# facebook/transform360

Hardware: NVIDIA H100
Metric: Mpixels/s 8K equirect->cubemap bicubic (input-plane pixels consumed per second) (higher is better)
Workload: dtype u8

## Files before the change

### include/transform360_b200.h

```cpp
#ifndef TRANSFORM360_B200_EXT_H
#define TRANSFORM360_B200_EXT_H

#include "Transform360/VideoFrameTransformHandler.h"

#ifdef __cplusplus
extern "C" {
#endif

typedef struct T360HostPlan T360HostPlan;

T360HostPlan* T360B200_hostPlanCreate(const FrameTransformContext* ctx, int inputWidth, int inputHeight,
                                      int outputWidth, int outputHeight);
#define T360_BORDER_WRAP 3
#define T360_BORDER_TRANSPARENT 5
T360HostPlan* T360B200_hostPlanCreateFromWarp(const FrameTransformContext* ctx, const float* map, int mapWidth, int mapHeight,
                                              int inputWidth, int inputHeight, int border);
void T360B200_hostPlanDestroy(T360HostPlan* plan);
int T360B200_hostPlanInfo(const T360HostPlan* plan, int info[6]);
const float* T360B200_hostPlanMap(const T360HostPlan* plan);
const int32_t* T360B200_hostPlanSamples(const T360HostPlan* plan);
int T360B200_hostPlanGather(T360HostPlan* plan, int info[10], const int32_t** jobs, const int32_t** records,
                            const uint32_t** compact);
int T360B200_hostPlanPoleCaps(T360HostPlan* plan, int info[4], const int32_t** capJobs, const uint32_t** capRecords,
                              const int32_t** launchJobs);
int T360B200_dealLanes(int interpolationAlg, int n, const int32_t* phases, int32_t* laneOf, int32_t* copyOf);
int T360B200_weightImage(int interpolationAlg, const uint8_t** image);
int T360B200_hostPlanBlurLists(T360HostPlan* const* plans, int numPlans, int width, int height, int layout[15],
                               const uint8_t** image);
int T360B200_hostPlanSegment(const T360HostPlan* plan, int i, int rect[4], int numTaps[2], const float** kx,
                             const float** ky);
int T360B200_remapTable(int interpolationAlg, const int16_t** table);

int T360B200_generateMapFromWarp(VideoFrameTransform* transform, const float* map, int mapWidth, int mapHeight, int inputWidth,
                                 int inputHeight, int border, int transformMatPlaneIndex);
int T360B200_remapFrameAsync(VideoFrameTransform* transform, int numPlanes, const float* const* deviceMaps, const int* mapPitches,
                             int border, const uint8_t* const* deviceInputs, uint8_t* const* deviceOutputs, const int* inputWidths,
                             const int* inputHeights, const int* inputPitches, const int* outputWidths, const int* outputHeights,
                             const int* outputPitches, void* cudaStream);

int T360B200_transformFramePlaneAsync(VideoFrameTransform* transform, const uint8_t* deviceInput,
                                      uint8_t* deviceOutput, int inputWidth, int inputHeight, int inputPitch,
                                      int outputWidth, int outputHeight, int outputPitch,
                                      int transformMatPlaneIndex, void* cudaStream);
int T360B200_transformFrameAsync(VideoFrameTransform* transform, int numPlanes, const uint8_t* const* deviceInputs,
                                 uint8_t* const* deviceOutputs, const int* inputWidths, const int* inputHeights,
                                 const int* inputPitches, const int* outputWidths, const int* outputHeights,
                                 const int* outputPitches, void* cudaStream);
int T360B200_lowPassPlaneAsync(VideoFrameTransform* transform, const uint8_t* deviceInput, uint8_t* deviceOutput,
                               int width, int height, int inputPitch, int outputPitch,
                               int transformMatPlaneIndex, void* cudaStream);
int T360B200_reconfigure(VideoFrameTransform* transform, const FrameTransformContext* ctx);
int T360B200_reconfigureAsync(VideoFrameTransform* transform, const FrameTransformContext* ctx);
int T360B200_reconfigureWait(VideoFrameTransform* transform, int block);
typedef struct T360View {
  float yaw, pitch, hfov, vfov;
} T360View;
int T360B200_transformFrameViewAsync(VideoFrameTransform* transform, const T360View* view, int numPlanes,
                                     const uint8_t* const* deviceInputs, uint8_t* const* deviceOutputs, const int* inputWidths,
                                     const int* inputHeights, const int* inputPitches, const int* outputWidths,
                                     const int* outputHeights, const int* outputPitches, void* cudaStream);
int T360B200_viewSamples(const FrameTransformContext* ctx, const T360View* view, int inputWidth, int inputHeight,
                         int outputWidth, int outputHeight, int32_t* samples);
typedef struct T360Orientation {
  float yaw, pitch, roll;
} T360Orientation;
int T360B200_transformFrameOrientedAsync(VideoFrameTransform* transform, const T360Orientation* orientation, int numPlanes,
                                         const uint8_t* const* deviceInputs, uint8_t* const* deviceOutputs,
                                         const int* inputWidths, const int* inputHeights, const int* inputPitches,
                                         const int* outputWidths, const int* outputHeights, const int* outputPitches,
                                         void* cudaStream);
int T360B200_orientedSamples(const FrameTransformContext* ctx, const T360Orientation* orientation, int inputWidth,
                             int inputHeight, int outputWidth, int outputHeight, int32_t* samples);
typedef struct T360Pose {
  float yaw, pitch, roll, hfov, vfov;
} T360Pose;
int T360B200_transformFramePoseAsync(VideoFrameTransform* transform, const T360Pose* pose, int numPlanes,
                                     const uint8_t* const* deviceInputs, uint8_t* const* deviceOutputs, const int* inputWidths,
                                     const int* inputHeights, const int* inputPitches, const int* outputWidths,
                                     const int* outputHeights, const int* outputPitches, void* cudaStream);
int T360B200_poseSamples(const FrameTransformContext* ctx, const T360Pose* pose, int inputWidth, int inputHeight,
                         int outputWidth, int outputHeight, int32_t* samples);
typedef struct T360Lens {
  float fx, fy, cx, cy;
  float k[4];
  float yaw, pitch, roll;
  float maxAngle;
} T360Lens;
typedef struct T360LensRig {
  int numLenses, calibWidth, calibHeight;
  T360Lens lens[2];
} T360LensRig;
int T360B200_lensMap(const FrameTransformContext* ctx, const T360LensRig* rig, const T360Orientation* orientation, int inputWidth,
                     int inputHeight, int outputWidth, int outputHeight, float* map);
int T360B200_transformFrameLensAsync(VideoFrameTransform* transform, const T360LensRig* rig, const T360Orientation* orientation,
                                     int numPlanes, const uint8_t* const* deviceInputs, uint8_t* const* deviceOutputs,
                                     const int* inputWidths, const int* inputHeights, const int* inputPitches,
                                     const int* outputWidths, const int* outputHeights, const int* outputPitches, void* cudaStream);
void T360B200_setPinHostPlanes(VideoFrameTransform* transform, int enable);
void T360B200_debugTrace(VideoFrameTransform* transform, int enable);
unsigned long long T360B200_debugTraceRead(VideoFrameTransform* transform, unsigned long long* out, unsigned long long maxWords);
int T360B200_synchronize(VideoFrameTransform* transform);
void* T360B200_stream(VideoFrameTransform* transform);

unsigned long long T360B200_kernelLaunchCount(void);
unsigned long long T360B200_planDeviceBytes(VideoFrameTransform* transform, int transformMatPlaneIndex);
int T360B200_planTileCounts(VideoFrameTransform* transform, int transformMatPlaneIndex, int counts[4]);
int T360B200_deviceCount(void);
const char* T360B200_version(void);

#ifdef __cplusplus
}
#endif
#endif
```

### transform360_b200/csrc/gather_frame.cu

```cuda
#include "gather_common.cuh"

#include <cuda.h>

#include <algorithm>
#include <cstring>
#include <utility>

namespace t360 {

namespace {

template <class F, int... I>
__device__ __forceinline__ void staticForImpl(F&& f, std::integer_sequence<int, I...>) {
  (f(std::integral_constant<int, I>{}), ...);
}
template <int N, class F>
__device__ __forceinline__ void staticFor(F&& f) {
  staticForImpl(f, std::make_integer_sequence<int, N>{});
}

template <int IMM>
__device__ __forceinline__ uint32_t ldsWordImm(uint32_t addr) {
  uint32_t v;
  asm volatile("ld.shared.u32 %0, [%1+%2];" : "=r"(v) : "r"(addr), "n"(IMM));
// ... 80 lines not shown
  }
  return acc;
}
template <int K>
__device__ __forceinline__ uint32_t slotOffset(uint32_t field) { return K == 2 ? field >> 1 : field; }

template <int VS>
__device__ __forceinline__ int foldRowsRotated(const RowBytes<8> (&W)[8], uint32_t wAddr, uint32_t field) {
  static_assert(VS == 16384, "one copy of the table");
  const uint32_t r = ((field >> 4) ^ threadIdx.x) & 7u;
  const uint32_t first = field ^ (r * (uint32_t)kDiagonalStep);
  const bool p0 = (r & 1u) != 0, p1 = (r & 2u) != 0, p2 = (r & 4u) != 0;
  RowBytes<8> A[8], B[8];
#pragma unroll
  for (int i = 0; i < 8; ++i)
#pragma unroll
    for (int h = 0; h < 2; ++h) A[i].b[h] = p0 ? W[i ^ 1].b[h] : W[i].b[h];
#pragma unroll
  for (int i = 0; i < 8; ++i)
#pragma unroll
    for (int h = 0; h < 2; ++h) B[i].b[h] = p1 ? A[i ^ 2].b[h] : A[i].b[h];
  int acc = 1 << 14;
  staticFor<8>([&](auto V) {
    constexpr int v = decltype(V)::value;
    const uint4 wt = ldsVecImm<0>(wAddr + (first ^ (uint32_t)(v * kDiagonalStep)));
    const uint32_t b0 = p2 ? B[v ^ 4].b[0] : B[v].b[0], b1 = p2 ? B[v ^ 4].b[1] : B[v].b[1];
    acc = dp2aLo(wt.x, b0, acc); acc = dp2aHi(wt.y, b0, acc);
    acc = dp2aLo(wt.z, b1, acc); acc = dp2aHi(wt.w, b1, acc);
  });
  return acc;
}
template <int K, int VS>
__device__ __forceinline__ int foldPixel(const RowBytes<K> (&W)[K], uint32_t wAddr, uint32_t field) {
  if constexpr (K == 8) return foldRowsRotated<VS>(W, wAddr, field);
  else return foldRows<K, VS>(W, wAddr + slotOffset<K>(field));
}
__device__ __forceinline__ int biasedToByte(int acc) { return min(max(acc >> 15, 0), 255); }


__device__ __forceinline__ uint32_t packBytes(int hi, int lo) {
  uint32_t r;
  asm("cvt.pack.sat.u8.s32.b32 %0, %1, %2, %3;" : "=r"(r) : "r"(hi), "r"(lo), "r"(0));
  return r;
}

template <int K, int PITCH, int VS, int ROWS, bool ZERO>
__device__ __forceinline__ void computeShareJob(uint8_t* dst, int dstPitch, uint32_t stageAddr, const uint4 (&rec)[ROWS / 8],
                                                uint32_t header, uint32_t wAddr) {
  static_assert(PITCH % 4 == 0 && (K == 4 || K == 8) && ROWS % 8 == 0, "");
  uint32_t base = stageAddr + (header & 0x7ffcu);
  const int sh = (int)(header << 3);
  RowBytes<K> W[K];
  staticFor<K>([&](auto R) { W[decltype(R)::value] = loadRow<K, decltype(R)::value * PITCH>(base, sh); });
  int accPrev = 0;
  staticFor<ROWS>([&](auto J) {
    constexpr int j = decltype(J)::value;
    const uint4& block = rec[j >> 3];
    const uint32_t word = ((j >> 1) & 3) == 0 ? block.x : (((j >> 1) & 3) == 1 ? block.y : (((j >> 1) & 3) == 2 ? block.z : block.w));
    const uint32_t r = (j & 1) ? word >> 16 : word;
    if constexpr (j > 0 && !ZERO) {
      const bool two = (r & 1u) != 0;
      const RowBytes<K> below = loadRow<K, (j - 1 + K) * PITCH>(base, sh);
      RowBytes<K> below2 = below;
      if (two) below2 = loadRow<K, (j + K) * PITCH>(base, sh);
#pragma unroll
      for (int q = 0; q + 2 < K; ++q)
#pragma unroll
        for (int i = 0; i < (K == 8 ? 2 : 1); ++i) W[q].b[i] = two ? W[q + 2].b[i] : W[q + 1].b[i];
#pragma unroll
      for (int i = 0; i < (K == 8 ? 2 : 1); ++i) W[K - 2].b[i] = two ? below.b[i] : W[K - 1].b[i];
      W[K - 1] = below2;
      if (two) base += PITCH;
    }
    if constexpr (j > 0 && ZERO) {
      const uint32_t d = r & 3u;
      RowBytes<K> below = W[K - 1], below2 = W[K - 1];
      if (d != 0) below = loadRow<K, K * PITCH>(base, sh);
      if (d == 2) below2 = loadRow<K, (K + 1) * PITCH>(base, sh);
#pragma unroll
      for (int q = 0; q + 2 < K; ++q)
#pragma unroll
        for (int i = 0; i < (K == 8 ? 2 : 1); ++i) W[q].b[i] = d == 0 ? W[q].b[i] : (d == 1 ? W[q + 1].b[i] : W[q + 2].b[i]);
#pragma unroll
      for (int i = 0; i < (K == 8 ? 2 : 1); ++i) {
        W[K - 2].b[i] = d == 0 ? W[K - 2].b[i] : (d == 1 ? W[K - 1].b[i] : below.b[i]);
        W[K - 1].b[i] = d == 0 ? W[K - 1].b[i] : (d == 1 ? below.b[i] : below2.b[i]);
      }
      base += d * PITCH;
    }
    const int acc = foldPixel<K, VS>(W, wAddr, r & kSlotFieldMask) >> 15;
    if constexpr (j & 1) {
      const uint32_t pair = packBytes(acc, accPrev);
      dst[(size_t)(j - 1) * dstPitch] = (uint8_t)pair;
      dst[(size_t)j * dstPitch] = (uint8_t)(pair >> 8);
    } else {
      accPrev = acc;
    }
  });
}

template <int K, int PITCH, int VS>
__device__ __forceinline__ void computeTileJob(const PlaneView& pv, uint32_t stageAddr, int outX, int outY, const uint4& rec,
                                               uint32_t wAddr, int warp) {
  static_assert(PITCH % 4 == 0, "");
  const int y0 = outY + warp * kTilePatchH;
  const int dstPitch = pv.dstPitch, dstW = pv.dstW, dstH = pv.dstH;
  uint8_t* const dstRow = pv.dst + (size_t)y0 * dstPitch + outX;
  const uint32_t words[4] = {rec.x, rec.y, rec.z, rec.w};
  staticFor<kRowsPerPatchStep>([&](auto J) {
    constexpr int j = decltype(J)::value;
    const uint32_t w = words[j];
    const int col = kTilePatchW * j + ((int)(w >> 16) & (kTilePatchW - 1)), row = (int)(w >> 19) & (kTilePatchH - 1);
    if (!(w & kRecordSkip) && outX + col < dstW && y0 + row < dstH) {
      const uint32_t rowAddr = stageAddr + (w & 0x7ffcu);
      const int sh = (int)(w << 3);
      RowBytes<K> W[K];
      staticFor<K>([&](auto R) { W[decltype(R)::value] = loadRow<K, decltype(R)::value * PITCH>(rowAddr, sh); });
      const int acc = foldPixel<K, VS>(W, wAddr, (w >> 17) & kSlotFieldMask);
      dstRow[(size_t)row * dstPitch + col] = (uint8_t)biasedToByte(acc);
    }
  });
}

template <int K, int PITCH, int VS>
__device__ __forceinline__ void computeCapJob(const PlaneView& pv, uint32_t stageAddr, uint32_t recAddr, int steps, uint32_t wAddr,
                                              int warp, int lane) {
  static_assert(PITCH % 4 == 0, "");
  for (int s = warp; s < steps; s += kGroupWarps) {
    const uint2 r = ldsVec2Imm<0>(recAddr + s * kCapStepBytes + lane * 8);
    if (r.x & kRecordSkip) continue;
    const uint32_t rowAddr = stageAddr + (r.x & 0x7ffcu);
    const int sh = (int)(r.x << 3);
    RowBytes<K> W[K];
    staticFor<K>([&](auto R) { W[decltype(R)::value] = loadRow<K, decltype(R)::value * PITCH>(rowAddr, sh); });
    const int acc = foldPixel<K, VS>(W, wAddr, (r.x >> 17) & kSlotFieldMask);
    pv.dst[(size_t)(r.y >> 16) * pv.dstPitch + (r.y & 0xffffu)] = (uint8_t)biasedToByte(acc);
  }
}

template <int K, int VS>
__device__ __forceinline__ void computeBorderJob(const PlaneView& pv, uint32_t recAddr, int n, const unsigned char* wsmem, int warp, int lane) {
  SrcView sv;
  sv.bytes = pv.src;
  sv.misalign = (int)(reinterpret_cast<uintptr_t>(pv.src) & 3);
  sv.words = reinterpret_cast<const uint32_t*>(pv.src - sv.misalign);
  sv.w = pv.srcW; sv.h = pv.srcH; sv.pitch = pv.srcPitch;
  for (int i = warp * 32 + lane; i < n; i += kGroupThreads) {
    const uint4 r = ldsVecImm<0>(recAddr + i * kBorderPixelBytes);
    const int v = gatherPixel<K, false, VS, weightDiagonal(K)>(sv, wsmem, (int)r.x, (int)r.y);
    pv.dst[(size_t)(r.z >> 16) * pv.dstPitch + (r.z & 0xffffu)] = (uint8_t)v;
  }
}

struct FrameTensorMaps {
  CUtensorMap map[kMaxFramePlanes][kNumBoxClasses][kBoxVariants];
};

__device__ __forceinline__ void mbarArrive(uint64_t* bar) {
  asm volatile("mbarrier.arrive.shared::cta.b64 _, [%0];" ::"r"(smemAddr(bar)) : "memory");
}
__device__ __forceinline__ uint4 ldsVec(uint32_t addr) {
  uint4 v;
  asm volatile("ld.shared.v4.u32 {%0, %1, %2, %3}, [%4];" : "=r"(v.x), "=r"(v.y), "=r"(v.z), "=r"(v.w) : "r"(addr));
  return v;
}
__device__ __forceinline__ uint32_t ldsWord(uint32_t addr) {
  uint32_t v;
  asm volatile("ld.shared.u32 %0, [%1];" : "=r"(v) : "r"(addr));
  return v;
}

template <int K, int COPIES, int GROUPS>
struct FrameLayout {
  static constexpr int kStages = gatherStages(K);
  static constexpr int kWeights = weightImageBytes(K, COPIES);
  static constexpr int kStage = stageBytesOf(K), kRec = stageRecordBytes(K);
  static constexpr int kGroupBytes = kStages * (kStage + kRec);
  static constexpr int kPlanes = kWeights + GROUPS * kGroupBytes;
  static constexpr int kBars = kPlanes + 256;
  static constexpr int kTotal = kBars + GROUPS * kStages * 16 + 16;
  static_assert(kTotal <= 232448, "227 KB of shared memory per CTA");
  static_assert(sizeof(PlaneView) * kMaxFramePlanes <= 256, "");
  static_assert(kStage % 128 == 0 && kRec % 128 == 0 && kWeights % 128 == 0, "TMA / bulk-copy destinations");
};

template <int K, int COPIES, int GROUPS>
__global__ void __launch_bounds__(GROUPS * (kGroupWarps + 1) * 32, 1)
gatherFrameKernel(const __grid_constant__ FrameGatherParams p, StagedParams jobs, const __grid_constant__ FrameTensorMaps maps) {
  using L = FrameLayout<K, COPIES, GROUPS>;
  constexpr int VS = weightVectorStride(K, COPIES), kStage = L::kStage, kRec = L::kRec, S = L::kStages;
  constexpr uint32_t kBox0 = stageBoxW(K, 0) * stageBoxH(K, 0), kBox1 = stageBoxW(K, 1) * stageBoxH(K, 1),
                     kBoxShare = stageBoxW(K, 2) * stageBoxH(K, 2);
  static_assert(kBox1 + 64 <= 2 * kStage && kBox0 + 64 <= kStage && kBoxShare + 64 <= kStage, "boxes must fit their stage buffers");
  static_assert(boxVariantRows(K, 0, kBoxVariants - 1) > 0 && boxVariantRows(K, 2, kBoxVariants - 1) > 0, "");
  extern __shared__ __align__(128) unsigned char smem[];
  unsigned char* wsmem = smem;
  PlaneView* planes = reinterpret_cast<PlaneView*>(smem + L::kPlanes);
  uint64_t* barBase = reinterpret_cast<uint64_t*>(smem + L::kBars);
  uint64_t* weightBar = barBase + GROUPS * 2 * S;
  const int warpId = threadIdx.x >> 5, lane = threadIdx.x & 31;
  constexpr int kProducerWarp = GROUPS * kGroupWarps;

  asm volatile("griddepcontrol.launch_dependents;" ::: "memory");
  if (threadIdx.x == 0) {
    for (int g = 0; g < GROUPS; ++g)
      for (int st = 0; st < S; ++st) {
        mbarInit(barBase + g * 2 * S + st, 1);
        mbarInit(barBase + g * 2 * S + S + st, kGroupWarps);
      }
    mbarInit(weightBar, 1);
    asm volatile("fence.mbarrier_init.release.cluster;" ::: "memory");
  }
  if (threadIdx.x < kMaxFramePlanes * (int)(sizeof(PlaneView) / 4))
    reinterpret_cast<uint32_t*>(planes)[threadIdx.x] = reinterpret_cast<const uint32_t*>(p.plane)[threadIdx.x];
  __syncthreads();

  if (warpId >= kProducerWarp) {
    const int g = warpId - kProducerWarp;
    if (g == 0 && lane == 0) {
      mbarExpectTx(weightBar, L::kWeights);
      constexpr int kChunk = L::kWeights / 4;
      for (int i = 0; i < 4; ++i)
        bulkCopyToShared(wsmem + i * kChunk, reinterpret_cast<const unsigned char*>(p.weightImage) + i * kChunk, kChunk, weightBar);
    }
    const int producer = blockIdx.x * GROUPS + g, dynamicBase = gridDim.x * GROUPS * 2 * kClaimBatch;
    auto loadBatch = [&](int base) {
      int4 h = make_int4(0, kJobExit << kJobKindShift, 0, 0);
      if (lane < kClaimBatch && base + lane < jobs.numTiles) h = __ldg(reinterpret_cast<const int4*>(jobs.tiles) + base + lane);
      return h;
    };
    int4 batch = loadBatch(producer * 2 * kClaimBatch);
    int4 batchNext = loadBatch((producer * 2 + 1) * kClaimBatch);
    asm volatile("griddepcontrol.wait;" ::: "memory");
    int claimed = 0;
    if (lane == 0) claimed = atomicAdd(jobs.claimCounter, kClaimBatch);
    unsigned char* groupBase = smem + L::kWeights + g * L::kGroupBytes;
    uint64_t* full = barBase + g * 2 * S;
    uint64_t* empty = full + S;
    int pos = 0;
    uint32_t st = 0, phase = 0;
    auto advance = [&]() { if (++st == S) { st = 0; phase ^= 1; } };
    auto postEmptyJob = [&](int kind) {
      *reinterpret_cast<int4*>(groupBase + S * kStage + st * kRec) = make_int4(0, kind << kJobKindShift, 0, 0);
      mbarArrive(full + st);
    };
    for (;;) {
      if (pos == kClaimBatch) {
        batch = batchNext;
        pos = 0;
        batchNext = loadBatch(dynamicBase + __shfl_sync(0xffffffffu, claimed, 0));
        if (lane == 0) claimed = atomicAdd(jobs.claimCounter, kClaimBatch);
      }
      int4 h;
      h.x = __shfl_sync(0xffffffffu, batch.x, pos); h.y = __shfl_sync(0xffffffffu, batch.y, pos);
      h.z = __shfl_sync(0xffffffffu, batch.z, pos); h.w = __shfl_sync(0xffffffffu, batch.w, pos);
      ++pos;
      const int kind = (h.y >> kJobKindShift) & kJobKindMask;
      mbarWait(empty + st, phase ^ 1);
      const bool twoStages = kind == kJobClass1 || kind == kJobSeam;
      if (twoStages) {
        if (st == S - 1) {
          if (lane == 0) postEmptyJob(kJobNop);
          advance();
          mbarWait(empty + st, phase ^ 1);
        }
        mbarWait(empty + st + 1, phase ^ 1);
      }
      if (lane == 0) {
        unsigned char* rec = groupBase + S * kStage + st * kRec;
        *reinterpret_cast<int4*>(rec) = h;
        if (kind == kJobExit) {
          mbarArrive(full + st);
        } else {
          const int pl = h.y >> kJobPlaneShift;
          const uint32_t recBytes = (uint32_t)jobRecordBytes(K, kind, h.x);
          if (kind == kJobBorder) {
            mbarExpectTx(full + st, recBytes);
          } else {
            const int cls = boxClassOf(kind), variant = jobBoxVariant(h.z), boxX = jobBoxX(h.z), boxY = jobBoxY(h.z);
            const uint32_t boxBytes = (uint32_t)(stageBoxW(K, cls) * boxVariantRows(K, cls, variant));
            mbarExpectTx(full + st, (kind == kJobSeam ? 2 : 1) * boxBytes + recBytes);
            tmaLoadBox(groupBase + st * kStage, &maps.map[pl][cls][variant], boxX, boxY, full + st);
            if (kind == kJobSeam)
              tmaLoadBox(groupBase + (st + 1) * kStage, &maps.map[pl][0][variant], boxX - planes[pl].srcW, boxY, full + st);
          }
          bulkCopyToShared(rec + 128, planes[pl].records + (unsigned)h.w, recBytes, full + st);
        }
      }
      advance();
      if (twoStages) {
        if (lane == 0) postEmptyJob(kJobNop);
        advance();
      }
      __syncwarp();
      if (kind == kJobExit) break;
    }
    if (lane == 0 && atomicAdd(jobs.claimCounter + 1, 1) == (int)(gridDim.x * GROUPS) - 1) {
      jobs.claimCounter[0] = 0;
      jobs.claimCounter[1] = 0;
      __threadfence();
    }
    return;
  }

  const int group = warpId / kGroupWarps, warp = warpId % kGroupWarps;
  unsigned char* groupBase = smem + L::kWeights + group * L::kGroupBytes;
  const uint32_t boxAddr = smemAddr(groupBase), recAddr = smemAddr(groupBase + S * kStage);
  uint64_t* full = barBase + group * 2 * S;
  uint64_t* empty = full + S;
  const uint32_t wAddr = smemAddr(wsmem);
  mbarWait(weightBar, 0);
  asm volatile("griddepcontrol.wait;" ::: "memory");
  auto now = []() { unsigned long long t; asm volatile("mov.u64 %0, %globaltimer;" : "=l"(t)); return t; };
  unsigned long long* trace = jobs.trace && warp == 0 && lane == 0 ? jobs.trace + (size_t)(blockIdx.x * GROUPS + group) * kTraceJobsPerGroup * 4 : nullptr;
  uint32_t traced = 0;
  for (uint32_t st = 0, phase = 0;;) {
    unsigned long long* const row = trace && traced < kTraceJobsPerGroup ? trace + traced * 4 : nullptr;
    if (row) row[0] = now();
    mbarWait(full + st, phase);
    if (row) row[1] = now();
    const uint32_t rec = recAddr + st * kRec;
    const uint4 h = ldsVec(rec);
    const int kind = ((int)h.y >> kJobKindShift) & kJobKindMask;
    if (kind == kJobExit) break;
    const int outX = (int)h.x & ~kJobQuadMask, outY = (int)h.y & kJobRowMask;
    const PlaneView& pv = planes[(int)h.y >> kJobPlaneShift];
    if (kind == kJobShare || kind == kJobShareStay) {
      if constexpr (K >= 4) {
        const uint32_t mine = rec + 128 + warp * shareWarpRecordBytes(K);
        uint4 r[shareRows(K) / 8];
#pragma unroll
        for (int b = 0; b < shareRows(K) / 8; ++b) r[b] = ldsVec(mine + b * 512 + lane * 16);
        const uint32_t header = ldsWord(mine + shareRows(K) / 8 * 512 + lane * 4);
        uint8_t* dst = pv.dst + (size_t)(outY + (warp >> 1) * shareRows(K)) * pv.dstPitch + (outX + (warp & 1) * 32 + (int)(header >> kRecordColumnShift));
        if (kind == kJobShare) computeShareJob<K, stageBoxW(K, 2), VS, shareRows(K), false>(dst, pv.dstPitch, boxAddr + st * kStage, r, header, wAddr);
        else computeShareJob<K, stageBoxW(K, 2), VS, shareRows(K), true>(dst, pv.dstPitch, boxAddr + st * kStage, r, header, wAddr);
      }
    } else if (kind == kJobClass0) {
      uint4 r;
      const int quad = ((int)h.x & kJobQuadMask) - 1;
      if (quad < 0) {
        r = ldsVec(rec + 128 + warp * 512 + lane * 16);
      } else {
        r = make_uint4(kRecordSkip, kRecordSkip, kRecordSkip, kRecordSkip);
        if ((warp >> 2) == (quad >> 1)) {
          const uint2 v = ldsVec2Imm<0>(rec + 128 + (warp & 3) * 256 + lane * 8);
          if (quad & 1) { r.z = v.x; r.w = v.y; } else { r.x = v.x; r.y = v.y; }
        }
      }
      computeTileJob<K, stageBoxW(K, 0), VS>(pv, boxAddr + st * kStage, outX, outY, r, wAddr, warp);
    } else if (kind == kJobClass1) {
      computeTileJob<K, stageBoxW(K, 1), VS>(pv, boxAddr + st * kStage, outX, outY, ldsVec(rec + 128 + warp * 512 + lane * 16), wAddr, warp);
    } else if (kind == kJobSeam) {
      {
        uint4* a = reinterpret_cast<uint4*>(groupBase + st * kStage);
        const uint4* b = reinterpret_cast<const uint4*>(groupBase + (st + 1) * kStage);
        for (int i = warp * 32 + lane; i < (int)(kBox0 / 16); i += kGroupThreads) {
          uint4 x = a[i];
          const uint4 y = b[i];
          x.x |= y.x; x.y |= y.y; x.z |= y.z; x.w |= y.w;
          a[i] = x;
        }
        asm volatile("fence.proxy.async.shared::cta;" ::: "memory");
      }
      groupBarrier(group);
      computeTileJob<K, stageBoxW(K, 0), VS>(pv, boxAddr + st * kStage, outX, outY, ldsVec(rec + 128 + warp * 512 + lane * 16), wAddr, warp);
    } else if (kind == kJobCap) {
      computeCapJob<K, stageBoxW(K, 0), VS>(pv, boxAddr + st * kStage, rec + 128, (int)h.x, wAddr, warp, lane);
    } else if (kind == kJobBorder) {
      computeBorderJob<K, VS>(pv, rec + 128, (int)h.x, wsmem, warp, lane);
    }
    __syncwarp();
    if (lane == 0) mbarArrive(empty + st);
    if (row) {
      row[2] = now(); row[3] = kind;
      ++traced;
    }
    if (++st == S) { st = 0; phase ^= 1; }
  }
}

template <int K, int COPIES, int GROUPS>
cudaError_t prepareFrameK(LaunchCfg& cfg) {
  static DeviceLaunchCfg cfgs;
  constexpr int threads = GROUPS * (kGroupWarps + 1) * 32, smemBytes = FrameLayout<K, COPIES, GROUPS>::kTotal;
  return prepare<gatherFrameKernel<K, COPIES, GROUPS>>(cfgs, threads, smemBytes, cfg);
}

template <int K, int COPIES, int GROUPS>
cudaError_t launchFrameK(const FrameGatherParams& p, const StagedParams& jobs, const FrameTensorMaps& maps, int numSMs,
                         cudaStream_t stream, bool programmatic) {
  constexpr int threads = GROUPS * (kGroupWarps + 1) * 32, smemBytes = FrameLayout<K, COPIES, GROUPS>::kTotal;
  LaunchCfg cfg;
  cudaError_t err = prepareFrameK<K, COPIES, GROUPS>(cfg);
  if (err != cudaSuccess) return err;
  const int grid = std::min(numSMs * cfg.perSM, (jobs.numTiles + GROUPS * 2 * kClaimBatch - 1) / (GROUPS * 2 * kClaimBatch));
  cudaLaunchConfig_t lc{};
  lc.gridDim = dim3(grid);
  lc.blockDim = dim3(threads);
  lc.dynamicSmemBytes = smemBytes;
  lc.stream = stream;
  cudaLaunchAttribute attr{};
  attr.id = cudaLaunchAttributeProgrammaticStreamSerialization;
  attr.val.programmaticStreamSerializationAllowed = 1;
  lc.attrs = &attr;
  lc.numAttrs = programmatic ? 1 : 0;
  err = cudaLaunchKernelEx(&lc, gatherFrameKernel<K, COPIES, GROUPS>, p, jobs, maps);
  gLaunches.fetch_add(1, std::memory_order_relaxed);
  return err;
}

}

cudaError_t prepareGatherFrame(int kernelSize) {
  LaunchCfg cfg;
  switch (kernelSize) {
    case 2: return prepareFrameK<2, weightCopies(2), gatherGroups(2)>(cfg);
    case 4: return prepareFrameK<4, weightCopies(4), gatherGroups(4)>(cfg);
    case 8: return prepareFrameK<8, weightCopies(8), gatherGroups(8)>(cfg);
    default: return cudaErrorInvalidValue;
  }
}

cudaError_t launchGatherFrame(const FrameGatherParams& p, const StagedParams& jobs, const void* tensorMaps, int numSMs,
                              cudaStream_t stream, bool programmatic) {
  if (jobs.numTiles <= 0) return cudaSuccess;
  if (p.numPlanes < 1 || p.numPlanes > kMaxFramePlanes) return cudaErrorInvalidValue;
  FrameTensorMaps maps;
  std::memcpy(&maps, tensorMaps, sizeof(CUtensorMap) * kNumBoxClasses * kBoxVariants * p.numPlanes);
  for (int i = p.numPlanes; i < kMaxFramePlanes; ++i)
    for (int c = 0; c < kNumBoxClasses; ++c)
      for (int v = 0; v < kBoxVariants; ++v) maps.map[i][c][v] = maps.map[0][c][v];
  switch (p.kernelSize) {
    case 2: return launchFrameK<2, weightCopies(2), gatherGroups(2)>(p, jobs, maps, numSMs, stream, programmatic);
    case 4: return launchFrameK<4, weightCopies(4), gatherGroups(4)>(p, jobs, maps, numSMs, stream, programmatic);
    case 8: return launchFrameK<8, weightCopies(8), gatherGroups(8)>(p, jobs, maps, numSMs, stream, programmatic);
    default: return cudaErrorInvalidValue;
  }
}

}
```

### transform360_b200/csrc/gather_plan.cpp

```cpp
#include "gather_plan.h"

#include <algorithm>
#include <climits>
#include <cstdint>
#include <cstring>
#include <stdexcept>
#include <thread>
#include <utility>

namespace t360 {
namespace {

template <class F>
void parallelRanges(int n, size_t workPerItem, F fn) {
  unsigned nt = std::thread::hardware_concurrency();
  if (nt == 0) nt = 1;
  if (nt > 32) nt = 32;
  if (static_cast<size_t>(n) * workPerItem < (1u << 16)) nt = 1;
  const int chunk = (n + static_cast<int>(nt) - 1) / static_cast<int>(nt);
  std::vector<std::thread> pool;
  for (unsigned t = 1; t < nt; ++t) {
    const int b = static_cast<int>(t) * chunk, e = std::min(n, b + chunk);
    if (b < e) pool.emplace_back(fn, b, e);
  }
// ... 433 lines not shown
    return false;
  }
  bool deal(const int* load) {
    std::memset(share, 0, sizeof(share));
    std::fill(fill, fill + 4, 0);
    for (int g = 0; g < groups; ++g)
      for (int i = 0; i < load[g]; ++i) {
        std::fill(seen, seen + 4, false);
        if (!put(g)) return false;
      }
    return true;
  }
};

int dealLanes(int k, int copies, int n, const int* slot, int* laneOf, int* copyOf) {
  const int groups = weightBankGroups(k), lanesPerPass = weightLanesPerPass(k), passes = 32 / lanesPerPass;
  for (int i = 0; i < n; ++i) { laneOf[i] = i; copyOf[i] = 0; }
  if (n < 32) return 0;
  int group[32];
  if (copies > 1 && groups == 8) {
    int base[32];
    for (int i = 0; i < n; ++i) base[i] = slot[i] & 7;
    GroupMatcher m{n, copies, 0, base, {}, {}, {}};
    for (m.cap = 4; m.cap <= 32; ++m.cap)
      if (m.run()) break;
    m.balance();
    for (int i = 0; i < n; ++i) {
      group[i] = m.groupOf[i];
      copyOf[i] = (m.groupOf[i] - base[i]) & 7;
    }
  } else {
    for (int i = 0; i < n; ++i) group[i] = slot[i] & (groups - 1);
  }
  int load[16] = {};
  for (int i = 0; i < n; ++i) ++load[group[i]];
  int share[16][4] = {}, height[4] = {};
  {
    int fullest = 0;
    for (int g = 0; g < groups; ++g) fullest = std::max(fullest, load[g]);
    PassDealer d{groups, passes, lanesPerPass, {}, {}, {}, {}};
    bool done = false;
    for (int total = std::max(passes, fullest); !done; ++total) {
      int h[4] = {1, 1, 1, 1};
      auto tryHeights = [&]() {
        std::copy(h, h + 4, d.h);
        if (!d.deal(load)) return false;
        std::memcpy(share, d.share, sizeof(share));
        std::copy(h, h + 4, height);
        return true;
      };
      if (passes == 2) {
        for (h[1] = total / 2; h[1] >= 1 && !done; --h[1]) { h[0] = total - h[1]; done = tryHeights(); }
      } else {
        for (h[3] = total / 4; h[3] >= 1 && !done; --h[3])
          for (h[2] = (total - h[3]) / 3; h[2] >= h[3] && !done; --h[2])
            for (h[1] = (total - h[3] - h[2]) / 2; h[1] >= h[2] && !done; --h[1]) {
              h[0] = total - h[3] - h[2] - h[1];
              done = tryHeights();
            }
      }
    }
  }
  int nextLane[4];
  for (int q = 0; q < passes; ++q) nextLane[q] = q * lanesPerPass;
  for (int g = 0; g < groups; ++g) {
    int q = 0;
    for (int i = 0; i < n; ++i) {
      if (group[i] != g) continue;
      while (share[g][q] == 0) ++q;
      --share[g][q];
      laneOf[i] = nextLane[q]++;
    }
  }
  int wavefronts = 0;
  for (int q = 0; q < passes; ++q) wavefronts += height[q];
  return wavefronts;
}

std::vector<uint8_t> buildWeightImage(int k, const int16_t* table) {
  const int copies = weightCopies(k);
  std::vector<uint8_t> img(static_cast<size_t>(weightImageBytes(k, copies)), 0);
  for (int phase = 0; phase < 1024; ++phase) {
    const int slot = weightSlotOf(k, phase);
    const int16_t* cell = table + static_cast<size_t>(phase) * k * k;
    if (k == 2) {
      std::memcpy(&img[static_cast<size_t>(slot) * 8], cell, 8);
      continue;
    }
    for (int c = 0; c < copies; ++c)
      for (int v = 0; v < k * k / 8; ++v)
        std::memcpy(&img[static_cast<size_t>(weightVectorOffset(k, copies, (weightSlotInCopy(slot, c) << 4) | (c << 14), v))], cell + v * 8, 16);
  }
  return img;
}

void buildGatherPlan(const HostPlan& h, bool stageTiles, GatherPlan& g) {
  g = GatherPlan{};
  const int k = h.kernelSize;
  if (k <= 0) return;
  g.tileH = gatherTileH(k);
  g.tilesPerRow = (h.mapW + kGatherTileW - 1) / kGatherTileW;
  g.tileRows = (h.mapH + g.tileH - 1) / g.tileH;
  g.records.assign(static_cast<size_t>(g.tilesPerRow) * g.tileRows * g.tileH * kGatherTileW, int2{0, 0});
  buildFullRecords(h, g.records, g.tilesPerRow, g.tileH);
  if (!stageTiles) return;

  const int tilesX = g.tilesPerRow, tilesY = (h.mapH + kFrameTileH - 1) / kFrameTileH;
  const bool seamPossible = h.inW % 16 == 0 && h.inW >= 4 * stageBoxW(k, 0);
  std::vector<TileClass> cls(static_cast<size_t>(tilesX) * tilesY);
  const int blockRows = shareH(k) / kFrameTileH;
  parallelRanges((tilesY + blockRows - 1) / blockRows, static_cast<size_t>(h.mapW) * shareH(k), [&](int byBegin, int byEnd) {
    for (int by = byBegin; by < byEnd; ++by)
      for (int tx = 0; tx < tilesX; tx += 2) {
        TileClass* c = &cls[static_cast<size_t>(by) * blockRows * tilesX + tx];
        if (shareBlock(h, tx * 32, by * shareH(k), c[0])) continue;
        for (int ty = by * blockRows; ty < std::min(tilesY, (by + 1) * blockRows); ++ty)
          for (int t = tx; t < std::min(tilesX, tx + 2); ++t)
            classifyTile(h, t * 32, ty * kFrameTileH, seamPossible, cls[static_cast<size_t>(ty) * tilesX + t]);
      }
  });

  for (int ty = 0; ty < tilesY; ++ty)
    for (int tx = 0; tx < tilesX; ++tx) {
      const TileClass& c = cls[static_cast<size_t>(ty) * tilesX + tx];
      const int kind = c.kind;
      if (kind < 0) continue;
      for (int q = 0; q < (c.quads ? 4 : 1); ++q) {
        GatherJob job{tx * 32, ty * kFrameTileH | (kind << kJobKindShift),
                      kind == kJobGeneral ? 0 : jobBoxField(c.boxX, c.boxY, boxVariantFor(k, boxClassOf(kind), c.boxRows)), 0};
        if (c.quads) {
          job.outX |= q + 1;
          job.boxXY = jobBoxField(c.quadBoxX[q], c.quadBoxY[q], boxVariantFor(k, 0, c.quadBoxRows[q]));
        }
        g.jobs.push_back(job);
      }
      switch (kind) {
        case kJobGeneral: ++g.numGeneral; break;
        case kJobSeam: ++g.numSeam; break;
        case kJobShare: case kJobShareStay: ++g.numShare; break;
        default: g.numStaged[kind] += c.quads ? 4 : 1; break;
      }
    }
  std::stable_sort(g.jobs.begin(), g.jobs.end(), [](const GatherJob& a, const GatherJob& b) { return jobLaunchRank(a) < jobLaunchRank(b); });
  size_t offset = 0;
  for (GatherJob& job : g.jobs) {
    const int kind = (job.outY >> kJobKindShift) & kJobKindMask;
    if (kind == kJobGeneral) continue;
    job.recordOffset = static_cast<int>(offset / 16);
    offset += jobRecordBytes(k, kind, job.outX);
  }
  g.compact.assign(offset / 4, 0u);
  std::vector<int> needRows(g.jobs.size(), h.inH);
  std::vector<JobRect> rects(g.jobs.size());
  parallelRanges(static_cast<int>(g.jobs.size()), 2048, [&](int begin, int end) {
    for (int i = begin; i < end; ++i) {
      const GatherJob& job = g.jobs[i];
      JobRect& r = rects[i];
      r = tileRect(job, k);
      r.x1 = std::min(r.x1, h.mapW);
      r.y1 = std::min(r.y1, h.mapH);
      const int kind = (job.outY >> kJobKindShift) & kJobKindMask;
      if (kind == kJobGeneral) continue;
      const Extent e = extentOf(h, r.x0, r.y0, r.x1, r.y1);
      if (e.minR >= 0 && e.maxR + k <= h.inH) needRows[i] = e.maxR + k;
      uint32_t* out = g.compact.data() + static_cast<size_t>(job.recordOffset) * 4;
      if (boxClassOf(kind) == 2) writeShareRecords(h, job, out);
      else writeTileRecords(h, job, out);
    }
  });

  std::vector<PixelJob> pixelJobs;
  coverPoleCaps(h, cls, tilesX, tilesY, pixelJobs);
  for (PixelJob& pj : pixelJobs) {
    const int kind = (pj.job.outY >> kJobKindShift) & kJobKindMask;
    pj.job.recordOffset = static_cast<int>(offset / 16);
    offset += jobRecordBytes(k, kind, pj.job.outX);
    g.capJobs.push_back(pj.job);
    g.capRecords.insert(g.capRecords.end(), pj.words.begin(), pj.words.end());
    ++(kind == kJobCap ? g.numCap : g.numBorder);
  }

  std::vector<int> launch;
  for (size_t i = 0; i < g.jobs.size(); ++i)
    if (((g.jobs[i].outY >> kJobKindShift) & kJobKindMask) != kJobGeneral) launch.push_back(static_cast<int>(i));
  for (size_t i = 0; i < g.capJobs.size(); ++i) launch.push_back(-1 - static_cast<int>(i));
  auto jobOf = [&](int i) -> const GatherJob& { return i >= 0 ? g.jobs[i] : g.capJobs[-1 - i]; };
  std::stable_sort(launch.begin(), launch.end(), [&](int a, int b) { return jobLaunchRank(jobOf(a)) < jobLaunchRank(jobOf(b)); });
  for (int i : launch) {
    g.launchJobs.push_back(jobOf(i));
    g.launchNeedRows.push_back(i >= 0 ? needRows[i] : pixelJobs[-1 - i].needRows);
    g.launchRects.push_back(i >= 0 ? rects[i] : pixelJobs[-1 - i].rect);
  }
}

}
```

### transform360_b200/csrc/gather_plan.h

```cpp
#pragma once

#include <cstdint>
#include <vector>

#include "host_plan.h"
#include "kernels.cuh"

namespace t360 {

struct JobRect {
  int x0, y0, x1, y1;
};

struct GatherPlan {
  int tilesPerRow = 0, tileRows = 0, tileH = 0;
  std::vector<int2> records;
  std::vector<GatherJob> jobs;
  std::vector<uint32_t> compact;
  std::vector<GatherJob> capJobs;
  std::vector<uint32_t> capRecords;
  std::vector<GatherJob> launchJobs;
  std::vector<int> launchNeedRows;
  std::vector<JobRect> launchRects;
  int numStaged[2] = {}, numSeam = 0, numGeneral = 0, numShare = 0, numCap = 0, numBorder = 0;
  int totalStaged() const { return numSeam + numShare + numStaged[0] + numStaged[1] + numCap; }
};

void buildGatherPlan(const HostPlan& h, bool stageTiles, GatherPlan& g);

inline int jobLaunchRank(const GatherJob& job) {
  switch ((job.outY >> kJobKindShift) & kJobKindMask) {
    case kJobBorder: case kJobGeneral: return 0;
    case kJobSeam: return 1;
    case kJobClass1: return 2;
    case kJobCap: return 3;
    case kJobShareStay: return 4;
    case kJobShare: return 5;
    default: return (job.outX & kJobQuadMask) ? 7 : 6;
  }
}


int dealLanes(int k, int copies, int n, const int* slot, int* laneOf, int* copyOf);

std::vector<uint8_t> buildWeightImage(int k, const int16_t* table);

}
```

### transform360_b200/csrc/kernels.cuh

```cuda
#pragma once

#include <cuda_runtime.h>

#include <cstdint>

#include "flat_view.h"
#include "oriented_view.h"

namespace t360 {

struct GatherParams {
  const uint8_t* src;
  int srcW, srcH, srcPitch;
  uint8_t* dst;
  int dstW, dstH, dstPitch;
  const int2* samples;
  int tilesPerRow;
  const int16_t* weights;
  int kernelSize;
  int transparent;
};

struct GatherJob {
  int outX, outY;
  int boxXY;
  int recordOffset;
};
constexpr int kBoxVariants = 3;
__host__ __device__ constexpr int jobBoxField(int boxX, int boxY, int variant) { return boxX | (boxY << 16) | variant; }
__host__ __device__ constexpr int jobBoxX(int boxXY) { return boxXY & 0xfff0; }
__host__ __device__ constexpr int jobBoxY(int boxXY) { return (int)((unsigned)boxXY >> 16); }
__host__ __device__ constexpr int jobBoxVariant(int boxXY) { return boxXY & 15; }
using StagedTile = GatherJob;
constexpr int kJobClass0 = 0, kJobClass1 = 1, kJobGeneral = 2, kJobShareStay = 3, kJobShare = 4, kJobNop = 5, kJobExit = 6, kJobSeam = 7,
              kJobCap = 8, kJobBorder = 9;
constexpr int kJobQuadMask = 7;
constexpr uint32_t kRecordSkip = 0x8000u;
constexpr int kJobKindShift = 24, kJobRowMask = (1 << kJobKindShift) - 1;
constexpr int kJobPlaneShift = 28, kJobKindMask = (1 << (kJobPlaneShift - kJobKindShift)) - 1;

constexpr int kGroupThreads = 256, kGroupWarps = kGroupThreads / 32;
__host__ __device__ constexpr int gatherGroups(int k) { return k == 8 ? 2 : 3; }
#ifndef T360_CLAIM_BATCH
#define T360_CLAIM_BATCH 1
#endif
constexpr int kClaimBatch = T360_CLAIM_BATCH;
constexpr int kGatherTileW = 32, kFrameTileH = 32;
constexpr int kTilePatchW = 8, kTilePatchH = 4, kRowsPerPatchStep = 4;
constexpr int kShareW = 64;
__host__ __device__ constexpr int shareRows(int ) { return 8; }
__host__ __device__ constexpr int shareH(int k) { return 4 * shareRows(k); }
constexpr int kNumBoxClasses = 3;
__host__ __device__ constexpr int boxClassOf(int kind) { return (kind == kJobShare || kind == kJobShareStay) ? 2 : (kind == kJobClass1 ? 1 : 0); }
__host__ __device__ constexpr int stageBoxW(int , int cls) { return cls == 2 ? 192 : (cls == 0 ? 208 : 240); }
__host__ __device__ constexpr int stageBoxH(int k, int cls) {
  return k == 8 ? (cls == 2 ? 80 : (cls == 0 ? 72 : 128)) : (cls == 2 ? 72 : (cls == 0 ? 64 : 96));
}
__host__ __device__ constexpr int boxVariantRows(int k, int cls, int v) {
  return cls == 1 || v == 0 ? stageBoxH(k, cls) : (cls == 2 ? stageBoxH(k, cls) - 8 * v : stageBoxH(k, cls) - 8 - 8 * v);
}
__host__ __device__ constexpr int boxVariantFor(int k, int cls, int rows) {
  int v = 0;
  while (v + 1 < kBoxVariants && cls != 1 && boxVariantRows(k, cls, v + 1) >= rows) ++v;
  return v;
}
__host__ __device__ constexpr int gatherStages(int ) { return 2; }
__host__ __device__ constexpr int stageBytesOf(int k) {
  const int a = stageBoxW(k, 2) * stageBoxH(k, 2), b = stageBoxW(k, 0) * stageBoxH(k, 0);
  return ((a > b ? a : b) + 64 + 127) & ~127;
}

__host__ __device__ constexpr int weightSlotOf(int k, int phase) {
  (void)k;
  return (phase & ~31) | ((phase & 1) << 4) | ((phase & 31) >> 1);
}
__host__ __device__ constexpr int weightCopies(int k) { return k == 4 ? 2 : 1; }
__host__ __device__ constexpr int weightVectorStride(int k, int copies) { return (k == 2 ? 8192 : 16384) * copies; }
__host__ __device__ constexpr int weightImageBytes(int k, int copies) { return k == 2 ? 8192 * copies : (k * k / 8) * 16384 * copies; }
__host__ __device__ constexpr int weightSlotInCopy(int slot, int copy) { return copy ? ((slot & ~7) | ((slot + copy) & 7)) : slot; }
__host__ __device__ constexpr int weightSlotField(int k, int phase, int copy) {
  return (weightSlotInCopy(weightSlotOf(k, phase), copy) << 4) | (copy << 14);
}
constexpr int kSlotFieldMask = 0x7FF0;
constexpr int kDiagonalStep = 0x4010;
__host__ __device__ constexpr bool weightDiagonal(int k) { return k == 8; }
__host__ __device__ constexpr int weightVectorOffset(int k, int copies, int slotFieldValue, int vector) {
  return weightDiagonal(k) ? (slotFieldValue ^ (vector * kDiagonalStep)) : slotFieldValue + vector * weightVectorStride(k, copies);
}
__host__ __device__ constexpr int weightBankGroups(int k) { return k == 2 ? 16 : 8; }
__host__ __device__ constexpr int weightLanesPerPass(int k) { return k == 2 ? 16 : 8; }

__host__ __device__ constexpr int shareWarpRecordBytes(int k) { return shareRows(k) / 8 * 32 * 16 + 32 * 4; }
__host__ __device__ constexpr int shareJobRecordBytes(int k) { return kGroupWarps * shareWarpRecordBytes(k); }
constexpr int kTileJobRecordBytes = kGroupWarps * 32 * 16;
constexpr int kQuadJobRecordBytes = kGroupWarps / 2 * 32 * 8;
__host__ __device__ constexpr int tileJobRecordBytes(int outXField) { return (outXField & kJobQuadMask) ? kQuadJobRecordBytes : kTileJobRecordBytes; }
__host__ __device__ constexpr int stageRecordBytes(int k) {
  return 128 + (shareJobRecordBytes(k) > kTileJobRecordBytes ? shareJobRecordBytes(k) : kTileJobRecordBytes);
}
constexpr int kCapStepBytes = 32 * 8, kBorderPixelBytes = 16;
__host__ __device__ constexpr int capJobMaxSteps(int k) { return (stageRecordBytes(k) - 128) / kCapStepBytes; }
__host__ __device__ constexpr int borderJobMaxPixels(int k) { return (stageRecordBytes(k) - 128) / kBorderPixelBytes; }
__host__ __device__ constexpr int jobRecordBytes(int k, int kind, int outXField) {
  return kind == kJobShare || kind == kJobShareStay ? shareJobRecordBytes(k)
         : kind == kJobCap                          ? outXField * kCapStepBytes
         : kind == kJobBorder                       ? outXField * kBorderPixelBytes
                                                    : tileJobRecordBytes(outXField);
}
constexpr int kRecordColumnShift = 27;

constexpr int kMaxFramePlanes = 3;
struct PlaneView {
  const uint8_t* src;
  uint8_t* dst;
  const uint4* records;
  int srcW, srcH, srcPitch;
  int dstW, dstH, dstPitch;
};
struct FrameGatherParams {
  PlaneView plane[kMaxFramePlanes];
  const uint4* weightImage;
  int kernelSize, numPlanes;
};

__host__ __device__ constexpr int gatherThreads(int k) { return k == 8 ? 512 : 256; }
__host__ __device__ constexpr int gatherTileH(int k) { return gatherThreads(k) / 32 * 4; }

struct StagedParams {
  const GatherJob* tiles;
  int numTiles;
  int* claimCounter;
  unsigned long long* trace;
};
constexpr int kTraceJobsPerGroup = 64;

struct BlurJob {
  int x0, y0, w, h;
  int kxOffset, kxCount, kyOffset, kyCount;
};

struct BlurParams {
  const uint8_t* src;
  uint8_t* dst;
  int width, height, srcPitch, dstPitch;
  const BlurJob* jobs;
  int numJobs;
  const float* taps;
  int tileSmemBytes;
};

struct StripJob {
  int x0, y0, w, h;
  int kxOffset, kxChunks, kxCount, kyOffset;
  int edge;
};

struct StripParams {
  const uint8_t* src;
  uint8_t* dst;
  int width, height, srcPitch, dstPitch;
  const StripJob* jobs;
  int numJobs;
  const float* taps;
};

struct AreaParams {
  const uint8_t* src;
  uint8_t* dst;
  int srcW, srcH, srcPitch, dstW, dstH, dstPitch;
  int cellW, cellH;
  const int2* xTaps;
  const int* xFirst;
  const int2* yTaps;
  const int* yFirst;
  const int2* xLinear;
  const int2* yLinear;
  int xMax;
};
cudaError_t launchAreaResize(const AreaParams& p, cudaStream_t stream);

struct FrameStripParams {
  struct Plane {
    const uint8_t* src;
    uint8_t* dst;
    int width, height, srcPitch, dstPitch;
  } plane[kMaxFramePlanes];
  int numPlanes;
  const StripJob* jobs;
  int numJobs;
  const float* taps;
};
constexpr int kStripPlaneShift = 8;
cudaError_t launchBlurFrameStrips(const FrameStripParams& p, int hy, cudaStream_t stream);

constexpr int kStripLanePx = 8, kStripW = 32 * kStripLanePx, kStripMaxHy = 3;

constexpr int kBlurTileW = 64, kBlurTileH = 32;
constexpr int kBlurMaxSmem = 96 * 1024;

cudaError_t launchGather(const GatherParams& p, int numSMs, cudaStream_t stream);
cudaError_t launchGatherFrame(const FrameGatherParams& p, const StagedParams& jobs, const void* tensorMaps, int numSMs,
                              cudaStream_t stream, bool programmatic = true);
cudaError_t prepareGatherFrame(int kernelSize);
cudaError_t launchBlur(const BlurParams& p, cudaStream_t stream);
cudaError_t launchBlurDirect(const BlurParams& p, cudaStream_t stream);
unsigned long long kernelLaunchCount();
void countKernelLaunches(long long n);

struct ViewPlane {
  const uint8_t* src;
  uint8_t* dst;
  int srcPitch, dstPitch;
  FlatGeometry geometry;
  int tilesX, firstTile;
};
struct ViewGatherParams {
  ViewPlane plane[kMaxFramePlanes];
  int numPlanes;
// ... 66 lines not shown
```

### transform360_b200/csrc/video_frame_transform.cpp

```cpp
#include <cuda.h>
#include <cuda_runtime.h>

#include <algorithm>
#include <chrono>
#include <climits>
#include <cmath>
#include <condition_variable>
#include <cstdarg>
#include <cstdio>
#include <cstdlib>
#include <cstring>
#include <map>
#include <memory>
#include <mutex>
#include <new>
#include <shared_mutex>
#include <stdexcept>
#include <string>
#include <string_view>
#include <thread>
#include <vector>

#include "host_plan.h"
#include "gather_plan.h"
#include "kernels.cuh"
#include "lowpass_jobs.h"
#include "transform360_b200.h"

#define T360_API extern "C" __attribute__((visibility("default")))

namespace {

using t360::BlurJob;
using t360::GatherJob;
using t360::HostPlan;
using t360::StripJob;

struct CudaFail {
  cudaError_t err;
  const char* what;
};

#define CU(call)                                       \
  do {                                                 \
    cudaError_t e__ = (call);                          \
    if (e__ != cudaSuccess) throw CudaFail{e__, #call}; \
  } while (0)

template <class Body>
bool guarded(std::string_view what, Body&& body) {
  const int n = static_cast<int>(what.size());
  try {
    return body();
  } catch (const CudaFail& f) {
    std::printf("%.*s. Error: CUDA %s (%s) in %s\n", n, what.data(), cudaGetErrorName(f.err), cudaGetErrorString(f.err), f.what);
    cudaGetLastError();
  } catch (const std::exception& ex) {
    std::printf("%.*s. Error: %s\n", n, what.data(), ex.what());
  }
  return false;
}

template <typename T>
struct DeviceBuffer {
  T* ptr = nullptr;
  size_t count = 0;
  DeviceBuffer() = default;
  DeviceBuffer(const DeviceBuffer&) = delete;
  DeviceBuffer& operator=(const DeviceBuffer&) = delete;
  DeviceBuffer(DeviceBuffer&& o) noexcept : ptr(o.ptr), count(o.count) { o.ptr = nullptr; o.count = 0; }
  DeviceBuffer& operator=(DeviceBuffer&& o) noexcept {
    if (this != &o) { release(); ptr = o.ptr; count = o.count; o.ptr = nullptr; o.count = 0; }
    return *this;
  }
  ~DeviceBuffer() { release(); }
  void release() {
    if (ptr) cudaFree(ptr);
    ptr = nullptr;
    count = 0;
  }
  void reserve(size_t n) {
    if (n <= count) return;
    release();
    CU(cudaMalloc(reinterpret_cast<void**>(&ptr), n * sizeof(T)));
    count = n;
  }
  size_t bytes() const { return count * sizeof(T); }
};

struct DevicePlan {
  int inW = 0, inH = 0, outW = 0, outH = 0, mapW = 0, mapH = 0;
  int kernelSize = 0;
  bool transparent = false, lowPass = false;
  bool warp = false;
  int stereoFormat = STEREO_FORMAT_MONO;
  DeviceBuffer<int2> samples;
  DeviceBuffer<uint32_t> records;
  int tilesPerRow = 0;
  DeviceBuffer<GatherJob> gatherJobs;
  std::vector<GatherJob> hostJobs;
  std::vector<int> jobNeedRows;
  std::vector<t360::JobRect> jobRects;
  int numJobs = 0, numStaged = 0, numBorder = 0;
  struct BlurSet {
    t360::BlurLists lists;
    t360::BlurLayout layout;
    DeviceBuffer<uint8_t> image;
    bool needsClear = false;
  };
  BlurSet blur;
  std::vector<t360::LowPassSegment> segments;
  std::vector<float> planTaps;
  mutable std::map<std::pair<int, int>, BlurSet> otherBlurs;
  struct Resize {
    int cellW = 0, cellH = 0, xMax = 0;
    DeviceBuffer<int2> xTaps, yTaps, xLinear, yLinear;
    DeviceBuffer<int> xFirst, yFirst;
  };
  bool resizeNeeded = false;
  mutable std::map<std::pair<int, int>, Resize> resizes;
  DeviceBuffer<float> sphereTables;
  size_t deviceBytes() const {
    return samples.bytes() + records.bytes() + gatherJobs.bytes() + blur.image.bytes();
  }
};

bool mergeable(const DevicePlan* const* plans, const t360::BlurLists* const* lists, const bool* clear, int numPlanes, const int* inW,
               const int* inH) {
  if (numPlanes < 2) return false;
  for (int p = 0; p < numPlanes; ++p) {
    const DevicePlan& d = *plans[p];
    if (d.transparent || inW[p] != d.inW || inH[p] != d.inH || clear[p] || !lists[p]->tiles.empty() || !lists[p]->direct.empty())
      return false;
  }
  return true;
}

struct HostIndexPlan {
  HostPlan host;
  t360::GatherPlan gather;
};
void gatherOnHost(HostIndexPlan& p) {
  if (p.host.kernelSize > 0) t360::buildGatherPlan(p.host, p.host.kernelSize >= 2 && !p.host.transparentBorder, p.gather);
}
bool planOnHost(const FrameTransformContext& ctx, int inW, int inH, int outW, int outH, HostIndexPlan& p) {
  if (!t360::buildHostPlan(ctx, inW, inH, outW, outH, p.host)) return false;
  gatherOnHost(p);
  return true;
}
bool planWarpOnHost(const FrameTransformContext& ctx, const float* map, int mapW, int mapH, int inW, int inH, int border, HostIndexPlan& p) {
  if (!t360::buildWarpHostPlan(ctx, map, mapW, mapH, inW, inH, border, p.host)) return false;
  gatherOnHost(p);
  return true;
}

void* driverEntry(const char* name) {
  void* p = nullptr;
  cudaDriverEntryPointQueryResult q{};
  if (cudaGetDriverEntryPoint(name, &p, cudaEnableDefault, &q) != cudaSuccess || q != cudaDriverEntryPointSuccess) {
    cudaGetLastError();
    p = nullptr;
  }
  return p;
}

constexpr std::chrono::milliseconds kSettleInterval{250};

using EncodeTiledFn = CUresult (*)(CUtensorMap*, CUtensorMapDataType, cuuint32_t, void*, const cuuint64_t*, const cuuint64_t*,
                                   const cuuint32_t*, const cuuint32_t*, CUtensorMapInterleave, CUtensorMapSwizzle,
                                   CUtensorMapL2promotion, CUtensorMapFloatOOBfill);

EncodeTiledFn tensorMapEncoder() {
  static const EncodeTiledFn fn = reinterpret_cast<EncodeTiledFn>(driverEntry("cuTensorMapEncodeTiled"));
  return fn;
}

bool encodePlaneMap(CUtensorMap* map, const uint8_t* base, int w, int h, int pitch, int k, int cls, int variant) {
  EncodeTiledFn enc = tensorMapEncoder();
  if (!enc) return false;
  if ((reinterpret_cast<uintptr_t>(base) & 15) || (pitch & 15)) return false;
  const cuuint64_t dims[2] = {static_cast<cuuint64_t>(w), static_cast<cuuint64_t>(h)};
  const cuuint64_t strides[1] = {static_cast<cuuint64_t>(pitch)};
  const cuuint32_t box[2] = {static_cast<cuuint32_t>(t360::stageBoxW(k, cls)), static_cast<cuuint32_t>(t360::boxVariantRows(k, cls, variant))};
  const cuuint32_t elem[2] = {1, 1};
  return enc(map, CU_TENSOR_MAP_DATA_TYPE_UINT8, 2, const_cast<uint8_t*>(base), dims, strides, box, elem,
             CU_TENSOR_MAP_INTERLEAVE_NONE, CU_TENSOR_MAP_SWIZZLE_NONE, CU_TENSOR_MAP_L2_PROMOTION_L2_128B,
             CU_TENSOR_MAP_FLOAT_OOB_FILL_NONE) == CUDA_SUCCESS;
}

constexpr int kPlaneLanes = 3;
static_assert(kPlaneLanes == t360::kMaxFramePlanes, "the frame kernel takes one PlaneView per lane");
struct PlaneMaps {
  const uint8_t* base = nullptr;
  int w = 0, h = 0, pitch = 0, k = 0;
  CUtensorMap maps[t360::kNumBoxClasses][t360::kBoxVariants];
};
struct PlaneLane {
  static constexpr int kMapCache = 32;
  PlaneMaps mapCache[kMapCache];
  int mapCacheNext = 0;
  cudaStream_t main = nullptr;
  cudaEvent_t done = nullptr;
  DeviceBuffer<uint8_t> blurred;
  DeviceBuffer<uint8_t> scaled;
  DeviceBuffer<int> claimCounter;
};

struct GatherWork {
  const DevicePlan* plan = nullptr;
  t360::PlaneView view{};
  bool staged = false;
  CUtensorMap maps[t360::kNumBoxClasses][t360::kBoxVariants];
  uint8_t* finalOut = nullptr;
  int finalPitch = 0, finalW = 0, finalH = 0, imagePlane = 0;
  const void* resizeTables = nullptr;
};

struct FrameLists {
  unsigned long long generation = ~0ull;
  DeviceBuffer<GatherJob> gatherJobs;
  int numGatherJobs = 0;
  DeviceBuffer<uint8_t> blurImage;
  t360::BlurLayout blurLayout;
};
struct FrameListRefs {
  const GatherJob* gatherJobs;
  int numGatherJobs;
  const uint8_t* blurImage;
  t360::BlurLayout blurLayout;
};

struct WavePlan {
  struct Rect { int x, y, w, h; };
  int chunks = 0;
  const void* plan = nullptr;
  unsigned long long generation = ~0ull;
  std::vector<int> chunkRowEnd, waveStart;
  DeviceBuffer<GatherJob> jobs;
  std::vector<std::vector<Rect>> rects;
};

struct PlaneGraph {
  const void* plan; unsigned long long generation; const void* in; const void* out; int inPitch, outPitch;
  const void* stagingIn; const void* stagingOut;
  int inW, inH, outW, outH;
  int kernels;
  cudaGraphExec_t exec; unsigned long long lastUse;
};

struct ViewBlurCache {
  std::vector<long long> key;
  bool merged = false;
  std::vector<uint8_t> jobs;
  std::vector<int> tapCodes;
  t360::BlurLayout layout[2];
  bool clear[2] = {false, false};
};

struct UploadRing {
  static constexpr int kEntries = 3;
  struct Entry {
    uint8_t* host = nullptr;
    uint8_t* device = nullptr;
    size_t capacity = 0;
    cudaEvent_t released = nullptr;
    bool inFlight = false;
  };
  Entry entries[kEntries];
  int last = -1;
  std::vector<uint8_t> lastContent;
};

struct StreamSlot {
  PlaneLane lanes[kPlaneLanes];
  DeviceBuffer<int> frameClaim;
  cudaEvent_t fork = nullptr;
  UploadRing viewJobs, viewTaps;
  ViewBlurCache viewBlur;
  UploadRing sphereTables;
  std::vector<uint8_t> sphereBytes;
  size_t sphereAt[kPlaneLanes] = {SIZE_MAX, SIZE_MAX, SIZE_MAX};
  FrameTransformContext sphereCtx{};
  std::vector<int> sphereSizes;
};

constexpr int kPitchAlign = 256;
inline int alignedPitch(int w) { return (w + kPitchAlign - 1) / kPitchAlign * kPitchAlign; }

struct FramePlanes {
  int numPlanes = 0;
  const uint8_t* in[kPlaneLanes];
  uint8_t* out[kPlaneLanes];
  int inW[kPlaneLanes], inH[kPlaneLanes], inPitch[kPlaneLanes], outW[kPlaneLanes], outH[kPlaneLanes], outPitch[kPlaneLanes];
};

bool describeFrame(const char* what, int numPlanes, const uint8_t* const* dIn, uint8_t* const* dOut, const int* inW, const int* inH,
                   const int* inPitch, const int* outW, const int* outH, const int* outPitch, FramePlanes& f) {
  if (!dIn || !dOut || !inW || !inH || !inPitch || !outW || !outH || !outPitch) {
    std::printf("%s. Error: a NULL argument\n", what);
    return false;
  }
  if (numPlanes < 1 || numPlanes > kPlaneLanes) {
    std::printf("%s. Error: %d planes (1..%d supported)\n", what, numPlanes, kPlaneLanes);
    return false;
  }
  f.numPlanes = numPlanes;
  for (int p = 0; p < numPlanes; ++p) {
    if (!dIn[p] || !dOut[p] || inW[p] <= 0 || inH[p] <= 0 || outW[p] <= 0 || outH[p] <= 0 || inPitch[p] < inW[p] || outPitch[p] < outW[p]) {
      std::printf("%s. Error: invalid description of plane %d\n", what, p);
      return false;
    }
    f.in[p] = dIn[p]; f.out[p] = dOut[p];
    f.inW[p] = inW[p]; f.inH[p] = inH[p]; f.inPitch[p] = inPitch[p];
    f.outW[p] = outW[p]; f.outH[p] = outH[p]; f.outPitch[p] = outPitch[p];
  }
  return true;
}

void setPose(FrameTransformContext& ctx, const T360Pose& pose) {
  ctx.fixed_yaw = pose.yaw;
  ctx.fixed_pitch = pose.pitch;
  ctx.fixed_roll = pose.roll;
  ctx.fixed_hfov = pose.hfov;
  ctx.fixed_vfov = pose.vfov;
}

std::string formatted(const char* fmt, ...) __attribute__((format(printf, 1, 2)));
std::string formatted(const char* fmt, ...) {
  char buf[320];
  va_list args;
  va_start(args, fmt);
  std::vsnprintf(buf, sizeof(buf), fmt, args);
  va_end(args);
  return buf;
}

std::string withFields(FrameTransformContext& ctx, const T360Pose& pose) {
  if (!std::isfinite(pose.yaw) || !std::isfinite(pose.pitch) || !std::isfinite(pose.roll) || !std::isfinite(pose.hfov) ||
      !std::isfinite(pose.vfov))
    return formatted("the pose (yaw %g, pitch %g, roll %g, hfov %g, vfov %g) is not finite", pose.yaw, pose.pitch, pose.roll, pose.hfov,
                     pose.vfov);
  if (ctx.output_layout < 0 || ctx.output_layout >= LAYOUT_N) return formatted("output_layout %d is not a layout", static_cast<int>(ctx.output_layout));
  setPose(ctx, pose);
  return {};
}
std::string withFields(FrameTransformContext& ctx, const T360View& view) {
  if (!std::isfinite(view.yaw) || !std::isfinite(view.pitch) || !std::isfinite(view.hfov) || !std::isfinite(view.vfov))
    return formatted("the view (yaw %g, pitch %g, hfov %g, vfov %g) is not finite", view.yaw, view.pitch, view.hfov, view.vfov);
  if (ctx.output_layout != LAYOUT_FLAT_FIXED)
    return formatted("per-frame views need output_layout FLAT_FIXED (%d), the transform has %d", static_cast<int>(LAYOUT_FLAT_FIXED),
                     static_cast<int>(ctx.output_layout));
  setPose(ctx, T360Pose{view.yaw, view.pitch, ctx.fixed_roll, view.hfov, view.vfov});
  return {};
}
std::string withFields(FrameTransformContext& ctx, const T360Orientation& o) {
  if (!std::isfinite(o.yaw) || !std::isfinite(o.pitch) || !std::isfinite(o.roll))
    return formatted("the orientation (yaw %g, pitch %g, roll %g) is not finite", o.yaw, o.pitch, o.roll);
  if (!t360::orientedLayouts(ctx))
    return formatted("per-frame orientations need output_layout CUBEMAP_32, CUBEMAP_23_OFFCENTER, EAC_32 or EQUIRECT and input_layout "
                     "EQUIRECT or CUBEMAP_32, the transform has %d -> %d%s", static_cast<int>(ctx.input_layout),
                     static_cast<int>(ctx.output_layout),
                     ctx.output_layout == LAYOUT_FLAT_FIXED ? " (FLAT_FIXED views: T360B200_transformFrameViewAsync)" : "");
  setPose(ctx, T360Pose{o.yaw, o.pitch, o.roll, ctx.fixed_hfov, ctx.fixed_vfov});
  return {};
}
// ... 860 lines not shown
  }

  void enableTrace(bool on) { traceEnabled_ = on; }
  size_t readTrace(unsigned long long* out, size_t maxWords) {
    if (!trace_.ptr) return 0;
    if (!out) return trace_.count;
    const size_t n = std::min(maxWords, trace_.count);
    if (cudaMemcpy(out, trace_.ptr, n * sizeof(unsigned long long), cudaMemcpyDeviceToHost) != cudaSuccess) return 0;
    return n;
  }

  bool synchronize() {
    if (!deviceReady_) return true;
    return cudaStreamSynchronize(stream_) == cudaSuccess;
  }
  cudaStream_t stream() {
    try { const DeviceRestore restoreDevice = ensureDevice(); } catch (...) { return nullptr; }
    return stream_;
  }
  bool tileCounts(int planIndex, int counts[4]) {
    std::lock_guard<std::mutex> lock(mu_);
    auto it = plans_.find(planIndex);
    if (it == plans_.end()) return false;
    counts[0] = it->second.numStaged; counts[1] = it->second.numBorder;
    const t360::BlurLayout& b = it->second.blur.layout;
    counts[2] = b.numStrips[0] + b.numStrips[1] + b.numStrips[2];
    counts[3] = b.numTiles + b.numDirect;
    return true;
  }
  size_t planBytes(int planIndex) {
    std::lock_guard<std::mutex> lock(mu_);
    auto it = plans_.find(planIndex);
    return it == plans_.end() ? 0 : it->second.deviceBytes();
  }

 private:
  StreamSlot& slotFor(cudaStream_t s) {
    std::lock_guard<std::mutex> lock(slotMu_);
    std::unique_ptr<StreamSlot>& slot = slots_[s];
    if (!slot) {
      slot.reset(new StreamSlot);
      for (int i = 0; i < kPlaneLanes; ++i) {
        PlaneLane& l = slot->lanes[i];
        if (i > 0) CU(cudaStreamCreateWithFlags(&l.main, cudaStreamNonBlocking));
        CU(cudaEventCreateWithFlags(&l.done, cudaEventDisableTiming));
      }
      CU(cudaEventCreateWithFlags(&slot->fork, cudaEventDisableTiming));
    }
    return *slot;
  }

  struct DeviceRestore {
    int previous = -1;
    DeviceRestore() = default;
    DeviceRestore(const DeviceRestore&) = delete;
    DeviceRestore& operator=(const DeviceRestore&) = delete;
    DeviceRestore(DeviceRestore&& o) noexcept : previous(o.previous) { o.previous = -1; }
    ~DeviceRestore() { if (previous >= 0) cudaSetDevice(previous); }
  };
  DeviceRestore ensureDevice() {
    DeviceRestore guard;
    if (deviceReady_) {
      int current = device_;
      CU(cudaGetDevice(&current));
      if (current != device_) {
        CU(cudaSetDevice(device_));
        guard.previous = current;
      }
      return guard;
    }
    int n = 0;
    cudaError_t e = cudaGetDeviceCount(&n);
    if (e != cudaSuccess || n <= 0) throw CudaFail{e != cudaSuccess ? e : cudaErrorNoDevice, "cudaGetDeviceCount (no CUDA device: this library has no CPU fallback)"};
    CU(cudaGetDevice(&device_));
    cudaDeviceProp prop{};
    CU(cudaGetDeviceProperties(&prop, device_));
    numSMs_ = prop.multiProcessorCount;
    CU(cudaStreamCreateWithFlags(&stream_, cudaStreamNonBlocking));
    if (auto getCurrent = reinterpret_cast<CUresult (*)(CUcontext*)>(driverEntry("cuCtxGetCurrent"))) getCurrent(&cuContext_);
    deviceReady_ = true;
    return guard;
  }

  void pinIfRecurring(const void* ptr, size_t bytes) {
    if (!pinHostPlanes_ || !ptr || !bytes) return;
    cudaPointerAttributes a{};
    if (cudaPointerGetAttributes(&a, ptr) != cudaSuccess) { cudaGetLastError(); return; }
    if (a.type != cudaMemoryTypeUnregistered) return;
    const uintptr_t page = 4096, lo = reinterpret_cast<uintptr_t>(ptr) & ~(page - 1);
    const size_t len = ((reinterpret_cast<uintptr_t>(ptr) + bytes + page - 1) & ~(page - 1)) - lo;
    for (HostRange& r : hostRanges_) {
      if (r.base != lo || r.bytes != len) continue;
      if (!r.pinned && ++r.seen >= 2) {
        if (cudaHostRegister(reinterpret_cast<void*>(lo), len, cudaHostRegisterDefault) == cudaSuccess) r.pinned = true;
        else { cudaGetLastError(); r.seen = -1000000; }
      }
      return;
    }
    if (hostRanges_.size() < 64) hostRanges_.push_back(HostRange{lo, len, 1, false});
  }

  static bool isDevicePointer(const void* p) {
    cudaPointerAttributes a{};
    if (cudaPointerGetAttributes(&a, p) != cudaSuccess) {
      cudaGetLastError();
      return false;
    }
    return a.type == cudaMemoryTypeDevice || a.type == cudaMemoryTypeManaged;
  }

  const DevicePlan* findPlan(int planIndex, int imagePlaneIndex) {
    std::lock_guard<std::mutex> lock(mu_);
    auto it = plans_.find(planIndex);
    if (it == plans_.end()) {
      std::printf("Could not transform the plane %d. Error: no map was generated for index %d\n", imagePlaneIndex, planIndex);
      return nullptr;
    }
    return &it->second;
  }

  const int16_t* deviceWeights(int interpolationAlg) {
    const int16_t* host = nullptr;
    const int k = t360::remapTable(interpolationAlg, &host);
    if (k < 2) return nullptr;
    std::lock_guard<std::mutex> lock(lazyMu_);
    auto& buf = weights_[k];
    if (!buf.ptr) {
      buf.reserve(static_cast<size_t>(1024) * k * k);
      CU(cudaMemcpy(buf.ptr, host, buf.bytes(), cudaMemcpyHostToDevice));
      const std::vector<uint8_t> image = t360::buildWeightImage(k, host);
      weightImages_[k].reserve(image.size());
      CU(cudaMemcpy(weightImages_[k].ptr, image.data(), image.size(), cudaMemcpyHostToDevice));
    }
    return buf.ptr;
  }

  DevicePlan upload(HostIndexPlan& p, const FrameTransformContext& ctx) {
    const HostPlan& h = p.host;
    DevicePlan d;
    d.inW = h.inW; d.inH = h.inH; d.outW = h.outW; d.outH = h.outH; d.mapW = h.mapW; d.mapH = h.mapH;
    d.kernelSize = h.kernelSize;
    d.transparent = h.transparentBorder;
    d.warp = h.warp;
    d.stereoFormat = ctx.input_stereo_format;
    if (d.kernelSize > 0) {
      deviceWeights(ctx.interpolation_alg);
      t360::GatherPlan& g = p.gather;
      d.tilesPerRow = g.tilesPerRow;
      d.samples.reserve(g.records.size());
      CU(cudaMemcpy(d.samples.ptr, g.records.data(), g.records.size() * sizeof(int2), cudaMemcpyHostToDevice));
      d.numStaged = g.totalStaged();
      d.numBorder = g.numBorder;
      d.numJobs = static_cast<int>(g.launchJobs.size());
      if (!g.launchJobs.empty()) {
        d.gatherJobs.reserve(g.launchJobs.size());
        CU(cudaMemcpy(d.gatherJobs.ptr, g.launchJobs.data(), g.launchJobs.size() * sizeof(GatherJob), cudaMemcpyHostToDevice));
      }
      if (!g.compact.empty() || !g.capRecords.empty()) {
        d.records.reserve(g.compact.size() + g.capRecords.size());
        if (!g.compact.empty())
          CU(cudaMemcpy(d.records.ptr, g.compact.data(), g.compact.size() * sizeof(uint32_t), cudaMemcpyHostToDevice));
        if (!g.capRecords.empty())
          CU(cudaMemcpy(d.records.ptr + g.compact.size(), g.capRecords.data(), g.capRecords.size() * sizeof(uint32_t), cudaMemcpyHostToDevice));
      }
      d.hostJobs = std::move(g.launchJobs);
      d.jobNeedRows = std::move(g.launchNeedRows);
      d.jobRects = std::move(g.launchRects);
    }
    d.lowPass = ctx.enable_low_pass_filter != 0;
    if (d.lowPass) {
      d.segments = h.segments;
      d.planTaps = h.taps;
      buildBlurSet(d.segments, d.planTaps, h.inW, h.inH, d.stereoFormat, d.blur);
    }
    d.resizeNeeded = h.resize.needed;
    if (d.resizeNeeded) resizeFor(d, d.outW, d.outH);
    if (d.kernelSize > 0 && !d.warp && ctx.output_layout != LAYOUT_FLAT_FIXED) {
      const std::vector<float> t = t360::buildSphereTables(t360::sphereGeometry(ctx, h.mapW, h.mapH, h.inW, h.inH, h.kernelSize));
      if (!t.empty()) {
        d.sphereTables.reserve(t.size());
        CU(cudaMemcpy(d.sphereTables.ptr, t.data(), t.size() * sizeof(float), cudaMemcpyHostToDevice));
      }
    }
    return d;
  }

  const DevicePlan::Resize& resizeFor(const DevicePlan& plan, int outW, int outH) {
    std::lock_guard<std::mutex> lock(lazyMu_);
    auto it = plan.resizes.find({outW, outH});
    if (it != plan.resizes.end()) return it->second;
    t360::AreaResizePlan r;
    t360::buildAreaResize(plan.mapW, plan.mapH, outW, outH, r);
    DevicePlan::Resize& d = plan.resizes[{outW, outH}];
    auto upload2 = [](const std::vector<int2>& v, DeviceBuffer<int2>& buf) {
      buf.reserve(std::max<size_t>(v.size(), 1));
      if (!v.empty()) CU(cudaMemcpy(buf.ptr, v.data(), v.size() * sizeof(int2), cudaMemcpyHostToDevice));
    };
    if (r.enlarge) {
      d.cellW = d.cellH = -1;
      d.xMax = r.lx.dmax;
      auto pack = [](const t360::AreaLinearAxis& a) {
        std::vector<int2> v(a.ofs.size());
        for (size_t i = 0; i < a.ofs.size(); ++i)
          v[i] = int2{a.ofs[i], static_cast<int>(static_cast<uint16_t>(a.coef[2 * i]) | (static_cast<uint32_t>(static_cast<uint16_t>(a.coef[2 * i + 1])) << 16))};
        return v;
      };
      upload2(pack(r.lx), d.xLinear);
      upload2(pack(r.ly), d.yLinear);
    } else if (r.cellW > 0) {
      d.cellW = r.cellW; d.cellH = r.cellH;
    } else {
      auto uploadAxis = [&](const t360::AreaAxis& a, DeviceBuffer<int2>& taps, DeviceBuffer<int>& first) {
        std::vector<int2> packed(a.taps.size());
        for (size_t i = 0; i < a.taps.size(); ++i) {
          int bits;
          std::memcpy(&bits, &a.taps[i].alpha, sizeof(bits));
          packed[i] = int2{a.taps[i].src, bits};
        }
        upload2(packed, taps);
        first.reserve(a.first.size());
        CU(cudaMemcpy(first.ptr, a.first.data(), a.first.size() * sizeof(int), cudaMemcpyHostToDevice));
      };
      uploadAxis(r.x, d.xTaps, d.xFirst);
      uploadAxis(r.y, d.yTaps, d.yFirst);
    }
    return d;
  }

  void buildBlurSet(const std::vector<t360::LowPassSegment>& segments, const std::vector<float>& planTaps, int planeW, int planeH,
                    int stereoFormat, DevicePlan::BlurSet& d) {
    t360::buildBlurLists(segments, planTaps, planeW, planeH, stereoFormat, d.lists, &d.needsClear);
    std::vector<uint8_t> image;
    d.layout = t360::packBlurLists(d.lists, image, image);
    if (image.empty()) return;
    d.image.reserve(image.size());
    CU(cudaMemcpy(d.image.ptr, image.data(), image.size(), cudaMemcpyHostToDevice));
  }

  const DevicePlan::BlurSet& blurFor(const DevicePlan& plan, int w, int h) {
    if (w == plan.inW && h == plan.inH) return plan.blur;
    std::lock_guard<std::mutex> lock(lazyMu_);
    auto it = plan.otherBlurs.find({w, h});
    if (it != plan.otherBlurs.end()) return it->second;
    DevicePlan::BlurSet& set = plan.otherBlurs[{w, h}];
    buildBlurSet(plan.segments, plan.planTaps, w, h, plan.stereoFormat, set);
    return set;
  }

  void launchLowPass(const t360::BlurLayout& l, bool clear, const uint8_t* jobs, const uint8_t* taps, t360::FrameStripParams fp, int numPlanes,
                     cudaStream_t s) {
    const t360::FrameStripParams::Plane& a = fp.plane[0];
    if (clear)
      for (int p = 0; p < numPlanes; ++p) CU(cudaMemset2DAsync(fp.plane[p].dst, fp.plane[p].dstPitch, 0, fp.plane[p].width, fp.plane[p].height, s));
    fp.numPlanes = numPlanes;
    fp.taps = reinterpret_cast<const float*>(taps + l.tapAt);
    for (int c = 0; c < t360::kStripMaxHy; ++c) {
      if (!l.numStrips[c]) continue;
      fp.jobs = reinterpret_cast<const StripJob*>(jobs + l.stripAt[c]);
      fp.numJobs = l.numStrips[c];
      CU(t360::launchBlurFrameStrips(fp, c + 1, s));
    }
    t360::BlurParams bp{a.src, a.dst, a.width, a.height, a.srcPitch, a.dstPitch, reinterpret_cast<const BlurJob*>(jobs + l.tileAt), l.numTiles,
                        fp.taps, l.tileSmem};
    if (bp.numJobs) CU(t360::launchBlur(bp, s));
    if (l.numDirect) {
      bp.jobs = reinterpret_cast<const BlurJob*>(jobs + l.directAt);
      bp.numJobs = l.numDirect;
      CU(t360::launchBlurDirect(bp, s));
    }
  }

  void runLowPass(const DevicePlan& plan, const uint8_t* dIn, uint8_t* dOut, int w, int h, int inPitch, int outPitch,
                  cudaStream_t s) {
    const DevicePlan::BlurSet& b = blurFor(plan, w, h);
    t360::FrameStripParams fp{};
    fp.plane[0] = {dIn, dOut, w, h, inPitch, outPitch};
    launchLowPass(b.layout, b.needsClear, b.image.ptr, b.image.ptr, fp, 1, s);
  }

  static bool planeMaps(PlaneLane& lane, const uint8_t* src, int w, int h, int pitch, int k,
                        CUtensorMap (&out)[t360::kNumBoxClasses][t360::kBoxVariants]) {
    for (const PlaneMaps& e : lane.mapCache)
      if (e.base == src && e.w == w && e.h == h && e.pitch == pitch && e.k == k) {
        std::memcpy(out, e.maps, sizeof(e.maps));
        return true;
      }
    PlaneMaps fresh;
    for (int c = 0; c < t360::kNumBoxClasses; ++c)
      for (int v = 0; v < t360::kBoxVariants; ++v) {
        if (v > 0 && t360::boxVariantRows(k, c, v) == t360::boxVariantRows(k, c, 0)) {
          fresh.maps[c][v] = fresh.maps[c][0];
          continue;
        }
        if (!encodePlaneMap(&fresh.maps[c][v], src, w, h, pitch, k, c, v)) return false;
      }
    fresh.base = src; fresh.w = w; fresh.h = h; fresh.pitch = pitch; fresh.k = k;
    lane.mapCache[lane.mapCacheNext] = fresh;
    lane.mapCacheNext = (lane.mapCacheNext + 1) % PlaneLane::kMapCache;
    std::memcpy(out, fresh.maps, sizeof(fresh.maps));
    return true;
  }

  bool enqueue(const DevicePlan& plan, const uint8_t* dIn, uint8_t* dOut, int inW, int inH, int inPitch, int outW,
               int outH, int outPitch, cudaStream_t s, int imagePlaneIndex, PlaneLane& lane) {
    GatherWork w;
    if (!prepareGather(plan, dIn, dOut, inW, inH, inPitch, outW, outH, outPitch, s, imagePlaneIndex, lane, w)) return false;
    if (plan.kernelSize == 0) return true;
    gatherPlane(w, lane, s);
    finishGather(w, s);
    return true;
  }

  bool prepareGather(const DevicePlan& plan, const uint8_t* dIn, uint8_t* dOut, int inW, int inH, int inPitch, int outW,
                     int outH, int outPitch, cudaStream_t s, int imagePlaneIndex, PlaneLane& lane, GatherWork& w, bool blurDone = false) {
    w.plan = &plan;
    w.imagePlane = imagePlaneIndex;
    if (plan.kernelSize == 0) {
      std::printf("Could not find interpolation algorithm for plane %d", imagePlaneIndex);
      return true;
    }
    w.finalOut = dOut;
    w.finalPitch = outPitch;
    w.finalW = outW;
    w.finalH = outH;
    w.resizeTables = nullptr;
    if (outW != plan.mapW || outH != plan.mapH) {
      w.resizeTables = &resizeFor(plan, outW, outH);
      const int sp = alignedPitch(plan.mapW);
      lane.scaled.reserve(static_cast<size_t>(sp) * plan.mapH + 64);
      if (plan.transparent) CU(cudaMemset2DAsync(lane.scaled.ptr, sp, planIndexOf(plan) ? 128 : 0, plan.mapW, plan.mapH, s));
      dOut = lane.scaled.ptr;
      outPitch = sp;
      outW = plan.mapW;
      outH = plan.mapH;
    }
    const uint8_t* src = dIn;
    int srcPitch = inPitch;
    if (plan.lowPass) {
      const int bp = alignedPitch(inW);
      lane.blurred.reserve(static_cast<size_t>(bp) * inH + 64);
      if (!blurDone) runLowPass(plan, dIn, lane.blurred.ptr, inW, inH, inPitch, bp, s);
      src = lane.blurred.ptr;
      srcPitch = bp;
    }
    w.view = t360::PlaneView{src, dOut, reinterpret_cast<const uint4*>(plan.records.ptr), inW, inH, srcPitch, outW, outH, outPitch};
    w.staged = plan.numJobs > 0 && !plan.transparent && inW == plan.inW && inH == plan.inH;
    if (w.staged) w.staged = planeMaps(lane, src, inW, inH, srcPitch, plan.kernelSize, w.maps);
    return true;
  }

  static void armScheduler(DeviceBuffer<int>& counter, cudaStream_t s) {
    if (counter.ptr) return;
    counter.reserve(2);
    CU(cudaMemsetAsync(counter.ptr, 0, 2 * sizeof(int), s));
  }

  void gatherPlane(const GatherWork& w, PlaneLane& lane, cudaStream_t s) {
    const DevicePlan& plan = *w.plan;
    if (w.staged) {
      armScheduler(lane.claimCounter, s);
      t360::FrameGatherParams fp{};
      fp.plane[0] = w.view;
      fp.weightImage = reinterpret_cast<const uint4*>(weightImages_[plan.kernelSize].ptr);
      fp.kernelSize = plan.kernelSize;
      fp.numPlanes = 1;
      t360::StagedParams jobs{plan.gatherJobs.ptr, plan.numJobs, lane.claimCounter.ptr, nullptr};
      CU(t360::launchGatherFrame(fp, jobs, w.maps, numSMs_, s));
    } else {
      const t360::PlaneView& v = w.view;
      t360::GatherParams gp{v.src, v.srcW, v.srcH, v.srcPitch, v.dst, v.dstW, v.dstH, v.dstPitch, plan.samples.ptr, plan.tilesPerRow,
                            weights_[plan.kernelSize].ptr, plan.kernelSize, plan.transparent ? 1 : 0};
      CU(t360::launchGather(gp, numSMs_, s));
    }
  }

  void blurFrame(const DevicePlan* const* plans, const FramePlanes& f, PlaneLane* lanes, cudaStream_t s) {
    const FrameListRefs l = frameLists(plans, f.numPlanes);
    t360::FrameStripParams fp{};
    for (int p = 0; p < f.numPlanes; ++p) {
      const int bp = alignedPitch(f.inW[p]);
      lanes[p].blurred.reserve(static_cast<size_t>(bp) * f.inH[p] + 64);
      fp.plane[p] = {f.in[p], lanes[p].blurred.ptr, f.inW[p], f.inH[p], f.inPitch[p], bp};
    }
    launchLowPass(l.blurLayout, false, l.blurImage, l.blurImage, fp, f.numPlanes, s);
  }

  bool viewLowPass(const char* what, const FrameTransformContext& ctx, const DevicePlan* const* plans, const FramePlanes& f, StreamSlot& slot,
                   cudaStream_t s, const uint8_t** src, int* srcPitch) {
    const int numPlanes = f.numPlanes;
    const int indices = numPlanes > 1 ? 2 : 1;
    HostPlan h[2];
    std::vector<long long> key{static_cast<long long>(planGeneration_), numPlanes};
    for (int idx = 0; idx < indices; ++idx) {
      const DevicePlan& plan = *plans[idx];
      h[idx].ctx = ctx;
      h[idx].inW = plan.inW; h[idx].inH = plan.inH; h[idx].outW = plan.outW; h[idx].outH = plan.outH; h[idx].mapW = plan.mapW; h[idx].mapH = plan.mapH;
      if (!t360::buildLowPassPlan(h[idx])) {
        std::printf("%s. Error: no low-pass plan for index %d\n", what, idx);
        return false;
      }
      key.push_back(reinterpret_cast<intptr_t>(&plan));
      key.push_back(static_cast<long long>(h[idx].taps.size()));
      const std::vector<float>& taps = h[idx].taps;
      const t360::LowPassSegment* prev = nullptr;
      for (const t360::LowPassSegment& g : h[idx].segments) {
        const bool same = prev && g.kxCount == prev->kxCount && g.kyCount == prev->kyCount &&
                          std::memcmp(&taps[g.kxOffset], &taps[prev->kxOffset], sizeof(float) * g.kxCount) == 0 &&
                          std::memcmp(&taps[g.kyOffset], &taps[prev->kyOffset], sizeof(float) * g.kyCount) == 0;
        for (long long v : {g.left, g.top, g.width, g.height, g.kxOffset, g.kxCount, g.kyOffset, g.kyCount}) key.push_back(v);
        key.push_back(same);
        prev = &g;
      }
    }
    ViewBlurCache& c = slot.viewBlur;
    std::vector<uint8_t> taps;
    if (c.key == key) {
      taps.resize(c.tapCodes.size() * sizeof(float));
      float* t = reinterpret_cast<float*>(taps.data());
      for (size_t i = 0; i < c.tapCodes.size(); ++i) {
        const int code = c.tapCodes[i];
        t[i] = code ? h[(code >> t360::kTapPlaneShift) ? 1 : 0].taps[(code & ((1 << t360::kTapPlaneShift) - 1)) - 1] : 0.f;
      }
    } else {
      c = ViewBlurCache{};
      t360::BlurLists lists[2];
      for (int idx = 0; idx < indices; ++idx) {
        c.clear[idx] = plans[idx]->blur.needsClear;
        t360::buildBlurLists(h[idx].segments, h[idx].taps, plans[idx]->inW, plans[idx]->inH, plans[idx]->stereoFormat, lists[idx],
                             perFrameOnly_ ? &c.clear[idx] : nullptr);
      }
      const t360::BlurLists* perPlane[kPlaneLanes];
      bool clear[kPlaneLanes];
      for (int p = 0; p < numPlanes; ++p) {
        perPlane[p] = &lists[p ? 1 : 0];
        clear[p] = c.clear[p ? 1 : 0];
      }
      c.merged = mergeable(plans, perPlane, clear, numPlanes, f.inW, f.inH);
      auto appendCodes = [&](const t360::BlurLists& l, const t360::BlurLayout& at, int plane) {
        c.tapCodes.resize(taps.size() / sizeof(float), 0);
        for (size_t i = 0; i < l.tapSource.size(); ++i)
          c.tapCodes[at.tapAt / sizeof(float) + i] = l.tapSource[i] ? (plane << t360::kTapPlaneShift) | l.tapSource[i] : 0;
      };
      if (c.merged) {
        const t360::BlurLists all = t360::mergeBlurLists(perPlane, numPlanes);
        c.layout[0] = t360::packBlurLists(all, c.jobs, taps);
        appendCodes(all, c.layout[0], 0);
      } else {
        for (int idx = 0; idx < indices; ++idx) {
          c.layout[idx] = t360::packBlurLists(lists[idx], c.jobs, taps);
          appendCodes(lists[idx], c.layout[idx], idx);
        }
      }
      c.key = std::move(key);
    }
    UploadRing::Entry* used[2];
    const uint8_t* dJobs = stageUpload(slot.viewJobs, c.jobs, s, &used[0]);
    const uint8_t* dTaps = stageUpload(slot.viewTaps, taps, s, &used[1]);
    t360::FrameStripParams fp{};
    for (int p = 0; p < numPlanes; ++p) {
      const int bp = alignedPitch(f.inW[p]);
      slot.lanes[p].blurred.reserve(static_cast<size_t>(bp) * f.inH[p] + 64);
      src[p] = slot.lanes[p].blurred.ptr;
      srcPitch[p] = bp;
      fp.plane[p] = {f.in[p], slot.lanes[p].blurred.ptr, f.inW[p], f.inH[p], f.inPitch[p], bp};
    }
    if (c.merged) {
      launchLowPass(c.layout[0], false, dJobs, dTaps, fp, numPlanes, s);
    } else {
      for (int p = 0; p < numPlanes; ++p) {
        t360::FrameStripParams one{};
        one.plane[0] = fp.plane[p];
        launchLowPass(c.layout[p ? 1 : 0], c.clear[p ? 1 : 0], dJobs, dTaps, one, 1, s);
      }
    }
    for (UploadRing::Entry* e : used) releaseAfter(e, s);
    return true;
  }

  static const uint8_t* stageUpload(UploadRing& ring, const std::vector<uint8_t>& bytes, cudaStream_t s, UploadRing::Entry** used) {
    if (ring.last >= 0 && ring.lastContent == bytes) {
      *used = &ring.entries[ring.last];
      return ring.entries[ring.last].device;
    }
    const int i = (ring.last + 1) % UploadRing::kEntries;
    UploadRing::Entry& e = ring.entries[i];
    ring.last = -1;
    if (!e.released) CU(cudaEventCreateWithFlags(&e.released, cudaEventDisableTiming));
    if (e.inFlight) CU(cudaEventSynchronize(e.released));
    e.inFlight = false;
    if (bytes.size() > e.capacity) {
      const size_t cap = std::max<size_t>(bytes.size() + bytes.size() / 4, 4096);
      if (e.host) CU(cudaFreeHost(e.host));
      e.host = nullptr;
      if (e.device) CU(cudaFreeAsync(e.device, s));
      e.device = nullptr;
      e.capacity = 0;
      CU(cudaHostAlloc(reinterpret_cast<void**>(&e.host), cap, cudaHostAllocDefault));
      CU(cudaMallocAsync(reinterpret_cast<void**>(&e.device), cap, s));
      e.capacity = cap;
    }
    if (!bytes.empty()) {
      std::memcpy(e.host, bytes.data(), bytes.size());
      CU(cudaMemcpyAsync(e.device, e.host, bytes.size(), cudaMemcpyHostToDevice, s));
    }
    ring.last = i;
    ring.lastContent = bytes;
    *used = &e;
    return e.device;
  }

  FrameListRefs frameLists(const DevicePlan* const* plans, int numPlanes) {
    std::lock_guard<std::mutex> lock(frameListsMu_);
    FrameLists& f = frameLists_[numPlanes - 2];
    if (f.generation != planGeneration_) {
      if (f.generation != ~0ull) CU(cudaDeviceSynchronize());
      buildFrameLists(plans, numPlanes, f);
      f.generation = planGeneration_;
    }
    return FrameListRefs{f.gatherJobs.ptr, f.numGatherJobs, f.blurImage.ptr, f.blurLayout};
  }

  void buildFrameLists(const DevicePlan* const* plans, int numPlanes, FrameLists& f) {
    std::vector<GatherJob> jobs;
    const t360::BlurLists* lists[kPlaneLanes];
    for (int p = 0; p < numPlanes; ++p) {
      for (GatherJob t : plans[p]->hostJobs) {
        t.outY |= p << t360::kJobPlaneShift;
        jobs.push_back(t);
      }
      lists[p] = &plans[p]->blur.lists;
    }
    std::stable_sort(jobs.begin(), jobs.end(), [](const GatherJob& a, const GatherJob& b) { return t360::jobLaunchRank(a) < t360::jobLaunchRank(b); });
    std::vector<uint8_t> image;
    const t360::BlurLayout layout = t360::packBlurLists(t360::mergeBlurLists(lists, numPlanes), image, image);
    f.gatherJobs.reserve(jobs.size());
    if (!jobs.empty()) CU(cudaMemcpy(f.gatherJobs.ptr, jobs.data(), jobs.size() * sizeof(GatherJob), cudaMemcpyHostToDevice));
    f.blurImage.reserve(image.size());
    if (!image.empty()) CU(cudaMemcpy(f.blurImage.ptr, image.data(), image.size(), cudaMemcpyHostToDevice));
    f.numGatherJobs = static_cast<int>(jobs.size());
    f.blurLayout = layout;
  }

  void gatherFrame(const GatherWork* work, int numPlanes, cudaStream_t s, StreamSlot& slot) {
    const DevicePlan* plans[kPlaneLanes];
    for (int p = 0; p < numPlanes; ++p) plans[p] = work[p].plan;
    const FrameListRefs f = frameLists(plans, numPlanes);
    armScheduler(slot.frameClaim, s);
    t360::FrameGatherParams fp{};
    CUtensorMap maps[kPlaneLanes][t360::kNumBoxClasses][t360::kBoxVariants];
    for (int p = 0; p < numPlanes; ++p) {
      fp.plane[p] = work[p].view;
      std::memcpy(maps[p], work[p].maps, sizeof(work[p].maps));
    }
    fp.weightImage = reinterpret_cast<const uint4*>(weightImages_[work[0].plan->kernelSize].ptr);
    fp.kernelSize = work[0].plan->kernelSize;
    fp.numPlanes = numPlanes;
    if (traceEnabled_) {
      trace_.reserve(static_cast<size_t>(numSMs_) * t360::gatherGroups(work[0].plan->kernelSize) * t360::kTraceJobsPerGroup * 4);
      CU(cudaMemsetAsync(trace_.ptr, 0, trace_.bytes(), s));
    }
    t360::StagedParams jobs{f.gatherJobs, f.numGatherJobs, slot.frameClaim.ptr, traceEnabled_ ? trace_.ptr : nullptr};
    CU(t360::launchGatherFrame(fp, jobs, maps, numSMs_, s));
  }

  void finishGather(const GatherWork& w, cudaStream_t s) {
    const DevicePlan& plan = *w.plan;
    if (!w.resizeTables) return;
    const DevicePlan::Resize& r = *static_cast<const DevicePlan::Resize*>(w.resizeTables);
    t360::AreaParams ap{w.view.dst, w.finalOut, plan.mapW, plan.mapH, w.view.dstPitch, w.finalW, w.finalH, w.finalPitch,
                        r.cellW, r.cellH, r.xTaps.ptr, r.xFirst.ptr, r.yTaps.ptr, r.yFirst.ptr, r.xLinear.ptr, r.yLinear.ptr, r.xMax};
    CU(t360::launchAreaResize(ap, s));
  }

  struct PlanSizes { int index, inW, inH, outW, outH; };
  std::vector<PlanSizes> plannedSizes() {
    std::lock_guard<std::mutex> lock(mu_);
    std::vector<PlanSizes> sizes;
    for (const auto& kv : plans_) sizes.push_back({kv.first, kv.second.inW, kv.second.inH, kv.second.outW, kv.second.outH});
    return sizes;
  }

  bool planesOfPlannedSize(const FramePlanes& f) {
    std::lock_guard<std::mutex> lock(mu_);
    for (int p = 0; p < f.numPlanes; ++p) {
      auto it = plans_.find(p ? 1 : 0);
      if (it != plans_.end() && (f.inW[p] != it->second.inW || f.inH[p] != it->second.inH)) return false;
    }
    return true;
  }

  bool refuseWarpPlans(const char* what) {
    std::lock_guard<std::mutex> lock(mu_);
    for (const auto& kv : plans_)
      if (kv.second.warp) {
        std::printf("%s. Error: plan index %d was generated from a warp map, which has no geometry to re-plan or to move "
                    "(generateMapForPlane on the index replaces it)\n", what, kv.first);
        return true;
      }
    return false;
  }

  std::shared_lock<std::shared_mutex> lockPlanned(const char* what) {
    for (;;) {
      std::shared_lock<std::shared_mutex> config(configMu_);
      if (!perFrameOnly_) return config;
      config.unlock();
      if (reconfigureWait(true) < 0) {
        std::printf("%s. Error: the background planner failed on the current context\n", what);
        return {};
      }
    }
  }

  static const char* asyncRefusal(const FrameTransformContext& next, const std::vector<PlanSizes>& sizes) {
    if (t360::kernelSizeOf(next.interpolation_alg) == 0) return "unknown interpolation_alg";
    for (float v : {next.input_expand_coef, next.expand_coef, next.width_scale_factor, next.height_scale_factor, next.fixed_yaw,
                    next.fixed_pitch, next.fixed_roll, next.fixed_hfov, next.fixed_vfov, next.fixed_cube_offcenter_x,
                    next.fixed_cube_offcenter_y, next.fixed_cube_offcenter_z, next.kernel_height_scale_factor, next.min_kernel_half_height,
                    next.max_kernel_half_height, next.kernel_adjust_factor})
      if (!std::isfinite(v)) return "a float field is not finite";
    if (!next.enable_low_pass_filter) return nullptr;
    if (next.num_vertical_segments < 1) return "num_vertical_segments must be positive";
    for (const PlanSizes& z : sizes) {
      HostPlan h;
      h.ctx = next;
      h.inW = z.inW; h.inH = z.inH; h.outW = z.outW; h.outH = z.outH;
      h.mapW = static_cast<int>(next.width_scale_factor * z.outW + 0.5);
      h.mapH = static_cast<int>(next.height_scale_factor * z.outH + 0.5);
      if (!t360::buildLowPassPlan(h)) return "the low-pass planner refuses the context";
    }
    return nullptr;
  }

  static bool planAll(const FrameTransformContext& next, const std::vector<PlanSizes>& sizes, std::vector<HostIndexPlan>& host,
                      const char* what) {
    host.assign(sizes.size(), HostIndexPlan{});
    std::vector<int> planned(sizes.size(), 0);
    std::vector<std::string> errors(sizes.size());
    auto planOne = [&](size_t i) {
      try {
        planned[i] = planOnHost(next, sizes[i].inW, sizes[i].inH, sizes[i].outW, sizes[i].outH, host[i]);
      } catch (const std::exception& ex) {
        errors[i] = ex.what();
      }
    };
    std::vector<std::thread> pool;
    for (size_t i = 1; i < sizes.size(); ++i) pool.emplace_back(planOne, i);
    planOne(0);
    for (std::thread& t : pool) t.join();
    for (size_t i = 0; i < sizes.size(); ++i)
      if (!planned[i]) {
        std::printf("%s. Error: no plan for index %d%s%s\n", what, sizes[i].index, errors[i].empty() ? "" : ": ", errors[i].c_str());
        return false;
      }
    return true;
  }

  struct PlanSet {
    std::map<int, DevicePlan> plans;
    FrameLists lists[kPlaneLanes - 1];
    std::vector<PlaneGraph> graphs;
  };
  PlanSet makePlanSet(const FrameTransformContext& next, const std::vector<PlanSizes>& sizes, std::vector<HostIndexPlan>& host) {
    PlanSet set;
    for (size_t i = 0; i < sizes.size(); ++i) set.plans.emplace(sizes[i].index, upload(host[i], next));
    auto luma = set.plans.find(0), chroma = set.plans.find(1);
    if (luma != set.plans.end() && chroma != set.plans.end()) {
      const DevicePlan* planes[kPlaneLanes] = {&luma->second, &chroma->second, &chroma->second};
      for (int n = 2; n <= kPlaneLanes; ++n) {
        buildFrameLists(planes, n, set.lists[n - 2]);
        set.lists[n - 2].generation = planGeneration_ + 1;
      }
    }
    return set;
  }

  bool install(PlanSet& set, const FrameTransformContext& next, unsigned long long seq, bool evenIfSuperseded) {
    std::unique_lock<std::shared_mutex> config(configMu_);
    std::lock_guard<std::mutex> async(asyncMu_);
    const bool current = asyncSeq_ == seq;
    if (!current && !evenIfSuperseded) return false;
    {
      std::lock_guard<std::mutex> lock(mu_);
      std::lock_guard<std::mutex> listsLock(frameListsMu_);
      plans_.swap(set.plans);
      for (int i = 0; i < kPlaneLanes - 1; ++i) std::swap(frameLists_[i], set.lists[i]);
      set.graphs.swap(planeGraphs_);
      ++planGeneration_;
    }
    if (current) {
      std::memcpy(&ctx_, &next, sizeof(ctx_));
      perFrameOnly_ = false;
      asyncSettled_ = seq;
      asyncFailed_ = false;
      asyncCv_.notify_all();
    }
    return true;
  }

  void retire(PlanSet& old) {
    CU(cudaDeviceSynchronize());
    for (PlaneGraph& g : old.graphs) cudaGraphExecDestroy(g.exec);
// ... 34 lines not shown
  }

  bool planPending(const FrameTransformContext& next, unsigned long long seq) {
    const char* what = "Could not reconfigure the transform in the background";
    auto superseded = [&] {
      std::lock_guard<std::mutex> async(asyncMu_);
      return asyncSeq_ != seq || asyncSettled_ == seq || asyncStop_;
    };
    return guarded(what, [&] {
      std::lock_guard<std::mutex> planLock(planMu_);
      if (superseded()) return true;
      const std::vector<PlanSizes> sizes = plannedSizes();
      std::vector<HostIndexPlan> host;
      if (!planAll(next, sizes, host, what)) return false;
      if (superseded()) return true;
      const DeviceRestore restoreDevice = ensureDevice();
      PlanSet set = makePlanSet(next, sizes, host);
      struct Retiring {
        VideoFrameTransform* t;
        explicit Retiring(VideoFrameTransform* self) : t(self) {
          std::lock_guard<std::mutex> async(t->asyncMu_);
          t->asyncRetiring_ = true;
        }
        ~Retiring() {
          std::lock_guard<std::mutex> async(t->asyncMu_);
          t->asyncRetiring_ = false;
          t->asyncCv_.notify_all();
        }
      } retiring(this);
      install(set, next, seq, false);
      retire(set);
      return true;
    });
  }

  void sphereTablesFor(const FrameTransformContext& ctx, int numPlanes, const int* mapW, const int* mapH, StreamSlot& slot, cudaStream_t s,
                       const float** tables, UploadRing::Entry** used) {
    FrameTransformContext key = ctx;
    key.fixed_yaw = key.fixed_pitch = key.fixed_roll = key.fixed_hfov = key.fixed_vfov = 0;
    std::vector<int> sizes;
    for (int p = 0; p < numPlanes; ++p) sizes.insert(sizes.end(), {mapW[p], mapH[p]});
    if (slot.sphereSizes != sizes || std::memcmp(&slot.sphereCtx, &key, sizeof(key)) != 0) {
      slot.sphereBytes.clear();
      for (int p = 0; p < numPlanes; ++p) {
        int same = 0;
        while (same < p && (mapW[same] != mapW[p] || mapH[same] != mapH[p])) ++same;
        if (same < p) {
          slot.sphereAt[p] = slot.sphereAt[same];
          continue;
        }
        const std::vector<float> t =
            t360::buildSphereTables(t360::sphereGeometry(ctx, mapW[p], mapH[p], 1, 1, t360::kernelSizeOf(ctx.interpolation_alg)));
        slot.sphereAt[p] = t.empty() ? SIZE_MAX : slot.sphereBytes.size();
        const uint8_t* bytes = reinterpret_cast<const uint8_t*>(t.data());
        slot.sphereBytes.insert(slot.sphereBytes.end(), bytes, bytes + t.size() * sizeof(float));
      }
      slot.sphereCtx = key;
      slot.sphereSizes = sizes;
    }
    for (int p = 0; p < numPlanes; ++p) tables[p] = nullptr;
    if (slot.sphereBytes.empty()) return;
    const uint8_t* d = stageUpload(slot.sphereTables, slot.sphereBytes, s, used);
    for (int p = 0; p < numPlanes; ++p) {
      const size_t at = slot.sphereAt[p];
      if (at != SIZE_MAX) tables[p] = reinterpret_cast<const float*>(d + at);
    }
  }

  int planIndexOf(const DevicePlan& plan) {
    std::lock_guard<std::mutex> lock(mu_);
    for (auto& kv : plans_)
      if (&kv.second == &plan) return kv.first;
    return 0;
  }

  FrameTransformContext ctx_;
  std::shared_mutex configMu_;
  std::mutex planMu_;
  std::mutex mu_;
  std::mutex lazyMu_;
  std::map<int, DevicePlan> plans_;
  DeviceBuffer<int16_t> weights_[9];
  DeviceBuffer<uint8_t> weightImages_[9];
  DeviceBuffer<uint8_t> stagingIn_, stagingOut_;
  std::mutex hostCallMu_;
  cudaStream_t copyIn_ = nullptr, copyIn2_ = nullptr, copyOut_ = nullptr;
  std::vector<cudaEvent_t> chunkIn_, waveDone_;
  WavePlan wavePlans_[2];
  long long pipelineMinBytes_ = 6ll << 20;
  int pipelineChunks_ = 0, pipelineBlocks_ = 0;
  int pipelineInStreams_ = 1;
  std::vector<PlaneGraph> planeGraphs_;
  unsigned long long graphClock_ = 0;
  cudaEvent_t graphFork_ = nullptr, graphJoinIn_ = nullptr, graphJoinOut_ = nullptr;
  struct HostRange { uintptr_t base; size_t bytes; int seen; bool pinned; };
  std::vector<HostRange> hostRanges_;
  bool pinHostPlanes_ = false;
  std::mutex slotMu_;
  std::map<cudaStream_t, std::unique_ptr<StreamSlot>> slots_;
  FrameLists frameLists_[kPlaneLanes - 1];
  std::mutex frameListsMu_;
  DeviceBuffer<unsigned long long> trace_;
  bool traceEnabled_ = false;
  unsigned long long planGeneration_ = 0;
  cudaStream_t stream_ = nullptr;
  int device_ = 0, numSMs_ = 0;
  bool deviceReady_ = false;
  CUcontext cuContext_ = nullptr;
  bool perFrameOnly_ = false;
  std::mutex asyncMu_;
  std::condition_variable asyncCv_;
  std::thread worker_;
  unsigned long long asyncSeq_ = 0, asyncSettled_ = 0;
  bool asyncFailed_ = false, asyncHurry_ = false, asyncStop_ = false;
  bool asyncRetiring_ = false;
  FrameTransformContext asyncCtx_{};
  std::chrono::steady_clock::time_point asyncLast_{};
};

T360_API VideoFrameTransform* VideoFrameTransform_new(FrameTransformContext* ctx) {
  if (!ctx) return nullptr;
  return new (std::nothrow) VideoFrameTransform(ctx);
}

T360_API void VideoFrameTransform_delete(VideoFrameTransform* transform) { delete transform; }

T360_API int VideoFrameTransform_generateMapForPlane(VideoFrameTransform* transform, int inputWidth, int inputHeight,
                                                     int outputWidth, int outputHeight, int transformMatPlaneIndex) {
  if (!transform) return 0;
  return transform->generateMapForPlane(inputWidth, inputHeight, outputWidth, outputHeight, transformMatPlaneIndex);
}

T360_API int T360B200_generateMapFromWarp(VideoFrameTransform* t, const float* map, int mapW, int mapH, int inW, int inH, int border,
                                          int planIndex) {
  if (!t) return 0;
  return t->generateMapFromWarp(map, mapW, mapH, inW, inH, border, planIndex);
}

T360_API int VideoFrameTransform_transformFramePlane(VideoFrameTransform* transform, uint8_t* inputData,
                                                     uint8_t* outputData, int inputWidth, int inputHeight,
                                                     int inputWidthWithPadding, int outputWidth, int outputHeight,
                                                     int outputWidthWithPadding, int transformMatPlaneIndex,
                                                     int imagePlaneIndex) {
  if (!transform) return 0;
  return transform->transformFramePlane(inputData, outputData, inputWidth, inputHeight, inputWidthWithPadding,
                                        outputWidth, outputHeight, outputWidthWithPadding, transformMatPlaneIndex,
                                        imagePlaneIndex);
}

struct T360HostPlan {
  HostPlan plan;
  t360::GatherPlan gather;
  bool gatherBuilt = false;
  std::vector<uint8_t> blurImage;
};

T360_API T360HostPlan* T360B200_hostPlanCreate(const FrameTransformContext* ctx, int inW, int inH, int outW, int outH) {
  if (!ctx) return nullptr;
  std::unique_ptr<T360HostPlan> p(new (std::nothrow) T360HostPlan);
  if (!p) return nullptr;
  try {
    if (!t360::buildHostPlan(*ctx, inW, inH, outW, outH, p->plan)) return nullptr;
  } catch (const std::exception& ex) {
    std::printf("Could not build the host plan. Error: %s\n", ex.what());
    return nullptr;
  }
  return p.release();
}
T360_API T360HostPlan* T360B200_hostPlanCreateFromWarp(const FrameTransformContext* ctx, const float* map, int mapW, int mapH, int inW,
                                                       int inH, int border) {
  if (!ctx) return nullptr;
  std::unique_ptr<T360HostPlan> p(new (std::nothrow) T360HostPlan);
  if (!p) return nullptr;
  try {
    if (!t360::buildWarpHostPlan(*ctx, map, mapW, mapH, inW, inH, border, p->plan)) return nullptr;
  } catch (const std::exception& ex) {
    std::printf("Could not build the host plan. Error: %s\n", ex.what());
    return nullptr;
  }
  return p.release();
}
T360_API void T360B200_hostPlanDestroy(T360HostPlan* plan) { delete plan; }
T360_API int T360B200_hostPlanInfo(const T360HostPlan* plan, int info[6]) {
  if (!plan || !info) return 0;
  info[0] = plan->plan.mapW; info[1] = plan->plan.mapH;
  info[2] = static_cast<int>(plan->plan.segments.size());
  info[3] = static_cast<int>(plan->plan.taps.size());
  info[4] = plan->plan.kernelSize;
  info[5] = 0;
  return 1;
}
T360_API const float* T360B200_hostPlanMap(const T360HostPlan* plan) { return plan ? plan->plan.map.data() : nullptr; }
T360_API const int32_t* T360B200_hostPlanSamples(const T360HostPlan* plan) {
  return plan && !plan->plan.samples.empty() ? reinterpret_cast<const int32_t*>(plan->plan.samples.data()) : nullptr;
}
T360_API int T360B200_hostPlanGather(T360HostPlan* plan, int info[10], const int32_t** jobs, const int32_t** records,
                                     const uint32_t** compact) {
  if (!plan || !info || plan->plan.kernelSize <= 0) return 0;
  try {
    if (!plan->gatherBuilt) {
      t360::buildGatherPlan(plan->plan, plan->plan.kernelSize >= 2 && !plan->plan.transparentBorder, plan->gather);
      plan->gatherBuilt = true;
    }
  } catch (const std::exception& ex) {
    std::printf("Could not build the gather plan. Error: %s\n", ex.what());
    return 0;
  }
  const t360::GatherPlan& g = plan->gather;
  info[0] = g.tilesPerRow; info[1] = g.tileRows; info[2] = g.tileH; info[3] = static_cast<int>(g.jobs.size());
  info[4] = g.numStaged[0]; info[5] = g.numStaged[1]; info[6] = g.numSeam; info[7] = g.numGeneral;
  info[8] = g.numShare; info[9] = static_cast<int>(g.compact.size());
  if (jobs) *jobs = g.jobs.empty() ? nullptr : reinterpret_cast<const int32_t*>(g.jobs.data());
  if (records) *records = reinterpret_cast<const int32_t*>(g.records.data());
  if (compact) *compact = g.compact.empty() ? nullptr : g.compact.data();
  return 1;
}
T360_API int T360B200_hostPlanPoleCaps(T360HostPlan* plan, int info[4], const int32_t** capJobs, const uint32_t** capRecords,
                                       const int32_t** launchJobs) {
  int gatherInfo[10];
  if (!plan || !info || !T360B200_hostPlanGather(plan, gatherInfo, nullptr, nullptr, nullptr)) return 0;
  const t360::GatherPlan& g = plan->gather;
  info[0] = g.numCap; info[1] = g.numBorder; info[2] = static_cast<int>(g.capRecords.size());
  info[3] = static_cast<int>(g.launchJobs.size());
  if (capJobs) *capJobs = g.capJobs.empty() ? nullptr : reinterpret_cast<const int32_t*>(g.capJobs.data());
  if (capRecords) *capRecords = g.capRecords.empty() ? nullptr : g.capRecords.data();
  if (launchJobs) *launchJobs = g.launchJobs.empty() ? nullptr : reinterpret_cast<const int32_t*>(g.launchJobs.data());
  return 1;
}
T360_API int T360B200_hostPlanBlurLists(T360HostPlan* const* plans, int numPlans, int width, int height, int layout[15],
                                        const uint8_t** image) {
  if (!plans || numPlans < 1 || numPlans > t360::kMaxFramePlanes || !layout || !image) return 0;
  for (int p = 0; p < numPlans; ++p)
    if (!plans[p]) return 0;
  try {
    t360::BlurLists lists[t360::kMaxFramePlanes];
    const t360::BlurLists* planes[t360::kMaxFramePlanes];
    bool clear = false;
    for (int p = 0; p < numPlans; ++p) {
      const HostPlan& h = plans[p]->plan;
      bool c = false;
      t360::buildBlurLists(h.segments, h.taps, width > 0 ? width : h.inW, height > 0 ? height : h.inH, h.ctx.input_stereo_format, lists[p], &c);
      clear = clear || c;
      planes[p] = &lists[p];
    }
    std::vector<uint8_t>& img = plans[0]->blurImage;
    img.clear();
    const t360::BlurLayout l = t360::packBlurLists(numPlans > 1 ? t360::mergeBlurLists(planes, numPlans) : lists[0], img, img);
    const long long v[15] = {l.numStrips[0], l.numStrips[1], l.numStrips[2], l.numTiles, l.numDirect, l.numTaps, l.tileSmem, clear,
                             static_cast<long long>(l.stripAt[0]), static_cast<long long>(l.stripAt[1]), static_cast<long long>(l.stripAt[2]),
                             static_cast<long long>(l.tileAt), static_cast<long long>(l.directAt), static_cast<long long>(l.tapAt),
                             static_cast<long long>(img.size())};
    for (int i = 0; i < 15; ++i) layout[i] = static_cast<int>(v[i]);
    *image = img.data();
    return 1;
  } catch (const std::exception& ex) {
    std::printf("Could not build the low-pass lists. Error: %s\n", ex.what());
    return 0;
  }
}
T360_API int T360B200_hostPlanSegment(const T360HostPlan* plan, int i, int rect[4], int numTaps[2], const float** kx,
                                      const float** ky) {
  if (!plan || i < 0 || i >= static_cast<int>(plan->plan.segments.size())) return 0;
  const t360::LowPassSegment& s = plan->plan.segments[i];
  rect[0] = s.left; rect[1] = s.top; rect[2] = s.width; rect[3] = s.height;
  numTaps[0] = s.kxCount; numTaps[1] = s.kyCount;
  if (kx) *kx = plan->plan.taps.data() + s.kxOffset;
  if (ky) *ky = plan->plan.taps.data() + s.kyOffset;
  return 1;
}
T360_API int T360B200_remapTable(int interpolationAlg, const int16_t** table) { return t360::remapTable(interpolationAlg, table); }
T360_API int T360B200_dealLanes(int interpolationAlg, int n, const int32_t* phases, int32_t* laneOf, int32_t* copyOf) {
  const int16_t* table = nullptr;
  const int k = t360::remapTable(interpolationAlg, &table);
  if (k < 2 || n < 0 || n > 32 || !phases || !laneOf || !copyOf) return -1;
  int slot[32], lane[32], copy[32];
  for (int i = 0; i < n; ++i) slot[i] = t360::weightSlotOf(k, phases[i] & 1023);
  const int wavefronts = t360::dealLanes(k, t360::weightCopies(k), n, slot, lane, copy);
  for (int i = 0; i < n; ++i) { laneOf[i] = lane[i]; copyOf[i] = copy[i]; }
  return wavefronts;
}

T360_API int T360B200_weightImage(int interpolationAlg, const uint8_t** image) {
  static std::mutex mu;
  static std::map<int, std::vector<uint8_t>> images;
  const int16_t* table = nullptr;
  const int k = t360::remapTable(interpolationAlg, &table);
  if (k < 2 || !image) return 0;
  std::lock_guard<std::mutex> lock(mu);
  auto it = images.find(k);
  if (it == images.end()) it = images.emplace(k, t360::buildWeightImage(k, table)).first;
  *image = it->second.data();
  return static_cast<int>(it->second.size());
}

T360_API int T360B200_transformFramePlaneAsync(VideoFrameTransform* t, const uint8_t* dIn, uint8_t* dOut, int inW, int inH,
                                               int inPitch, int outW, int outH, int outPitch, int planIndex, void* stream) {
  if (!t || !dIn || !dOut) return 0;
  return t->transformDevice(dIn, dOut, inW, inH, inPitch, outW, outH, outPitch, planIndex, static_cast<cudaStream_t>(stream));
}
T360_API int T360B200_transformFrameAsync(VideoFrameTransform* t, int numPlanes, const uint8_t* const* dIn, uint8_t* const* dOut,
                                          const int* inW, const int* inH, const int* inPitch, const int* outW, const int* outH,
                                          const int* outPitch, void* stream) {
  FramePlanes f;
  if (!t || !describeFrame("Could not transform the frame", numPlanes, dIn, dOut, inW, inH, inPitch, outW, outH, outPitch, f)) return 0;
  return t->transformFrameDevice(f, static_cast<cudaStream_t>(stream));
}
T360_API int T360B200_lowPassPlaneAsync(VideoFrameTransform* t, const uint8_t* dIn, uint8_t* dOut, int w, int h, int inPitch,
                                        int outPitch, int planIndex, void* stream) {
  if (!t || !dIn || !dOut) return 0;
  return t->lowPassDevice(dIn, dOut, w, h, inPitch, outPitch, planIndex, static_cast<cudaStream_t>(stream));
}
T360_API int T360B200_reconfigure(VideoFrameTransform* t, const FrameTransformContext* ctx) {
  if (!t || !ctx) return 0;
  return t->reconfigure(*ctx);
}
T360_API int T360B200_reconfigureAsync(VideoFrameTransform* t, const FrameTransformContext* ctx) {
  if (!t || !ctx) return 0;
  return t->reconfigureAsync(*ctx);
}
T360_API int T360B200_reconfigureWait(VideoFrameTransform* t, int block) {
  if (!t) return -1;
  return t->reconfigureWait(block != 0);
}
T360_API int T360B200_transformFrameViewAsync(VideoFrameTransform* t, const T360View* view, int numPlanes, const uint8_t* const* dIn,
                                              uint8_t* const* dOut, const int* inW, const int* inH, const int* inPitch, const int* outW,
                                              const int* outH, const int* outPitch, void* stream) {
  const char* what = "Could not transform the frame with a view";
  FramePlanes f;
  if (!t || !view || !describeFrame(what, numPlanes, dIn, dOut, inW, inH, inPitch, outW, outH, outPitch, f)) return 0;
  return t->transformFrameWith(what, *view, f, static_cast<cudaStream_t>(stream));
}
template <class Fields>
static int perFrameSamples(const char* what, const FrameTransformContext* context, const Fields* fields, int inW, int inH, int outW, int outH,
                           int32_t* samples) {
  if (!context || !fields || !samples) return 0;
  FrameTransformContext ctx = *context;
  const std::string why = withFields(ctx, *fields);
  if (!why.empty()) {
    std::printf("Could not compute the %s's samples. Error: %s\n", what, why.c_str());
    return 0;
  }
  const int k = t360::kernelSizeOf(ctx.interpolation_alg);
  const int mapW = static_cast<int>(ctx.width_scale_factor * outW + 0.5), mapH = static_cast<int>(ctx.height_scale_factor * outH + 0.5);
  if (k == 0 || inW <= 0 || inH <= 0 || outW <= 0 || outH <= 0 || mapW <= 0 || mapH <= 0) {
    std::printf("Could not compute the %s's samples. Error: invalid interpolation or plane sizes\n", what);
    return 0;
  }
  if (ctx.output_layout == LAYOUT_FLAT_FIXED) {
    const t360::FlatGeometry g = t360::flatGeometry(ctx, mapW, mapH, inW, inH, k);
    const t360::FlatView v{ctx.fixed_yaw, ctx.fixed_pitch, ctx.fixed_hfov, ctx.fixed_vfov};
    for (int i = 0; i < mapH; ++i)
      for (int j = 0; j < mapW; ++j) {
        int32_t* out = samples + 2 * (static_cast<size_t>(i) * mapW + j);
        t360::flatSample(v, g, i, j, out, out + 1);
      }
    return 1;
  }
  const t360::SphereGeometry g = t360::sphereGeometry(ctx, mapW, mapH, inW, inH, k);
  const std::vector<float> tables = t360::buildSphereTables(g);
  const float* colTab = tables.data();
  const float* rowTab = tables.empty() ? nullptr : tables.data() + t360::sphereTableRowOffset(g);
  const t360::Rotation r = t360::rotationFromAngles(ctx.fixed_yaw, ctx.fixed_pitch, ctx.fixed_roll);
  for (int i = 0; i < mapH; ++i)
    for (int j = 0; j < mapW; ++j) {
      int32_t* out = samples + 2 * (static_cast<size_t>(i) * mapW + j);
      t360::sphereSample(g, r, colTab, rowTab, i, j, out, out + 1);
    }
  return 1;
}

T360_API int T360B200_viewSamples(const FrameTransformContext* ctx, const T360View* view, int inW, int inH, int outW, int outH, int32_t* samples) {
  return perFrameSamples("view", ctx, view, inW, inH, outW, outH, samples);
}
T360_API int T360B200_transformFrameOrientedAsync(VideoFrameTransform* t, const T360Orientation* orientation, int numPlanes,
                                                  const uint8_t* const* dIn, uint8_t* const* dOut, const int* inW, const int* inH,
                                                  const int* inPitch, const int* outW, const int* outH, const int* outPitch, void* stream) {
  const char* what = "Could not transform the frame with an orientation";
  FramePlanes f;
  if (!t || !orientation || !describeFrame(what, numPlanes, dIn, dOut, inW, inH, inPitch, outW, outH, outPitch, f)) return 0;
// ... 88 lines not shown
```

### transform360_b200/handler.py

```python
from __future__ import annotations

import ctypes as C
import os
from pathlib import Path

import numpy as np

PKG = Path(__file__).resolve().parent
LIB_PATH = PKG / "lib" / "libTransform360.so"

LAYOUT_CUBEMAP_32, LAYOUT_CUBEMAP_23_OFFCENTER, LAYOUT_FLAT_FIXED, LAYOUT_EQUIRECT = 0, 1, 2, 3
LAYOUT_BARREL, LAYOUT_BARREL_SPLIT, LAYOUT_EAC_32, LAYOUT_N = 4, 5, 6, 7
STEREO_FORMAT_TB, STEREO_FORMAT_LR, STEREO_FORMAT_MONO, STEREO_FORMAT_GUESS, STEREO_FORMAT_N = 0, 1, 2, 3, 4
NEAREST, LINEAR, CUBIC, LANCZOS4 = 0, 1, 2, 4
BORDER_WRAP, BORDER_TRANSPARENT = 3, 5


def _warp_map(map) -> np.ndarray:
    m = np.ascontiguousarray(map, np.float32)
    if m.ndim != 3 or m.shape[2] != 2:
        raise ValueError(f"a warp map is float32 [h][w][2] (x, y per output pixel), got shape {m.shape}")
    return m


def _frame_args(in_planes, out_planes, dims):
    n = len(in_planes)
    VP, IA = C.c_void_p * n, C.c_int * n
    d_in = VP(*[p[0] for p in in_planes])
    d_out = VP(*[p[0] for p in out_planes])
    arrs = [IA(*[d[0] for d in dims]), IA(*[d[1] for d in dims]), IA(*[p[1] for p in in_planes]),
            IA(*[d[2] for d in dims]), IA(*[d[3] for d in dims]), IA(*[p[1] for p in out_planes])]
    ptrs = [C.cast(a, C.c_void_p) for a in arrs]
    return n, C.cast(d_in, C.c_void_p), C.cast(d_out, C.c_void_p), ptrs, (d_in, d_out, arrs)


def _samples(fn, ctx, fields, in_w, in_h, out_w, out_h) -> np.ndarray:
    scaled = lambda f, n: int(float(np.float32(f) * np.float32(n)) + 0.5)
    map_w, map_h = scaled(ctx.width_scale_factor, out_w), scaled(ctx.height_scale_factor, out_h)
    out = np.zeros((max(map_h, 0), max(map_w, 0), 2), np.int32)
    if not fn(C.byref(ctx), C.byref(fields), in_w, in_h, out_w, out_h, out.ctypes.data):
        raise ValueError(f"{fn.__name__} refused the arguments (message on stdout)")
    return out


class FrameTransformContext(C.Structure):
    _fields_ = [
        ("input_layout", C.c_int), ("output_layout", C.c_int),
        ("input_stereo_format", C.c_int), ("output_stereo_format", C.c_int),
        ("vflip", C.c_int), ("input_expand_coef", C.c_float), ("expand_coef", C.c_float),
        ("interpolation_alg", C.c_int), ("width_scale_factor", C.c_float),
        ("height_scale_factor", C.c_float), ("fixed_yaw", C.c_float), ("fixed_pitch", C.c_float),
        ("fixed_roll", C.c_float), ("fixed_hfov", C.c_float), ("fixed_vfov", C.c_float),
        ("fixed_cube_offcenter_x", C.c_float), ("fixed_cube_offcenter_y", C.c_float),
        ("fixed_cube_offcenter_z", C.c_float), ("is_horizontal_offset", C.c_int),
        ("enable_low_pass_filter", C.c_int), ("kernel_height_scale_factor", C.c_float),
        ("min_kernel_half_height", C.c_float), ("max_kernel_half_height", C.c_float),
        ("enable_multi_threading", C.c_int), ("num_vertical_segments", C.c_int),
        ("num_horizontal_segments", C.c_int), ("adjust_kernel", C.c_int),
        ("kernel_adjust_factor", C.c_float),
    ]


FILTER_DEFAULTS = dict(
    input_layout=LAYOUT_EQUIRECT, output_layout=LAYOUT_CUBEMAP_32, input_stereo_format=STEREO_FORMAT_MONO,
    output_stereo_format=STEREO_FORMAT_MONO, vflip=0, input_expand_coef=1.01, expand_coef=1.01,
    interpolation_alg=CUBIC, width_scale_factor=1.0, height_scale_factor=1.0, fixed_yaw=0.0, fixed_pitch=0.0,
    fixed_roll=0.0, fixed_hfov=120.0, fixed_vfov=110.0, fixed_cube_offcenter_x=0.0, fixed_cube_offcenter_y=0.0,
    fixed_cube_offcenter_z=0.0, is_horizontal_offset=0, enable_low_pass_filter=1, kernel_height_scale_factor=1.0,
    min_kernel_half_height=1.0, max_kernel_half_height=10000.0, enable_multi_threading=1, num_vertical_segments=5,
    num_horizontal_segments=1, adjust_kernel=1, kernel_adjust_factor=1.0)


class T360View(C.Structure):
    _fields_ = [("yaw", C.c_float), ("pitch", C.c_float), ("hfov", C.c_float), ("vfov", C.c_float)]


def as_view(view) -> T360View:
    return view if isinstance(view, T360View) else T360View(*[float(v) for v in view])


class T360Orientation(C.Structure):
    _fields_ = [("yaw", C.c_float), ("pitch", C.c_float), ("roll", C.c_float)]


def as_orientation(orientation) -> T360Orientation:
    if isinstance(orientation, T360Orientation):
        return orientation
    return T360Orientation(*[float(v) for v in orientation])


class T360Pose(C.Structure):
    _fields_ = [("yaw", C.c_float), ("pitch", C.c_float), ("roll", C.c_float), ("hfov", C.c_float), ("vfov", C.c_float)]


def as_pose(pose) -> T360Pose:
    return pose if isinstance(pose, T360Pose) else T360Pose(*[float(v) for v in pose])


class T360Lens(C.Structure):
    _fields_ = [("fx", C.c_float), ("fy", C.c_float), ("cx", C.c_float), ("cy", C.c_float), ("k", C.c_float * 4),
                ("yaw", C.c_float), ("pitch", C.c_float), ("roll", C.c_float), ("maxAngle", C.c_float)]


class T360LensRig(C.Structure):
    _fields_ = [("numLenses", C.c_int), ("calibWidth", C.c_int), ("calibHeight", C.c_int), ("lens", T360Lens * 2)]


def make_context(**overrides) -> FrameTransformContext:
    vals = dict(FILTER_DEFAULTS)
    for k in overrides:
        if k not in vals:
            raise AttributeError(f"FrameTransformContext has no field {k!r}")
    vals.update(overrides)
    return FrameTransformContext(**vals)


_lib = None


def load(path: os.PathLike | None = None):
    global _lib
    if _lib is not None and path is None:
        return _lib
    p = Path(path) if path else Path(os.environ.get("T360B200_LIB") or LIB_PATH)
    if not p.exists():
        raise FileNotFoundError(f"{p} not found: build it with `python -m transform360_b200.build` (needs nvcc); "
                                "transform360_b200 has no CPU fallback")
    L = C.CDLL(str(p), mode=os.RTLD_LOCAL)
    vp, ci = C.c_void_p, C.c_int
    L.VideoFrameTransform_new.restype = vp
    L.VideoFrameTransform_new.argtypes = [C.POINTER(FrameTransformContext)]
    L.VideoFrameTransform_delete.restype = None
    L.VideoFrameTransform_delete.argtypes = [vp]
    L.VideoFrameTransform_generateMapForPlane.restype = ci
    L.VideoFrameTransform_generateMapForPlane.argtypes = [vp] + [ci] * 5
    L.VideoFrameTransform_transformFramePlane.restype = ci
    L.VideoFrameTransform_transformFramePlane.argtypes = [vp, vp, vp] + [ci] * 8
    L.T360B200_hostPlanCreate.restype = vp
    L.T360B200_hostPlanCreate.argtypes = [C.POINTER(FrameTransformContext)] + [ci] * 4
    L.T360B200_hostPlanCreateFromWarp.restype = vp
    L.T360B200_hostPlanCreateFromWarp.argtypes = [C.POINTER(FrameTransformContext), vp] + [ci] * 5
    L.T360B200_generateMapFromWarp.restype = ci
    L.T360B200_generateMapFromWarp.argtypes = [vp, vp] + [ci] * 6
    L.T360B200_remapFrameAsync.restype = ci
    L.T360B200_remapFrameAsync.argtypes = [vp, ci, vp, vp, ci] + [vp] * 8 + [vp]
    L.T360B200_hostPlanDestroy.restype = None
    L.T360B200_hostPlanDestroy.argtypes = [vp]
    L.T360B200_hostPlanInfo.restype = ci
    L.T360B200_hostPlanInfo.argtypes = [vp, C.POINTER(ci)]
    L.T360B200_hostPlanMap.restype = vp
    L.T360B200_hostPlanMap.argtypes = [vp]
    L.T360B200_hostPlanSamples.restype = vp
    L.T360B200_hostPlanSamples.argtypes = [vp]
    L.T360B200_hostPlanSegment.restype = ci
    L.T360B200_hostPlanSegment.argtypes = [vp, ci, C.POINTER(ci), C.POINTER(ci), C.POINTER(vp), C.POINTER(vp)]
    L.T360B200_hostPlanGather.restype = ci
    L.T360B200_hostPlanGather.argtypes = [vp, C.POINTER(ci), C.POINTER(vp), C.POINTER(vp), C.POINTER(vp)]
    L.T360B200_hostPlanPoleCaps.restype = ci
    L.T360B200_hostPlanBlurLists.restype = ci
    L.T360B200_hostPlanBlurLists.argtypes = [vp, ci, ci, ci, C.POINTER(ci), C.POINTER(vp)]
    L.T360B200_hostPlanPoleCaps.argtypes = [vp, C.POINTER(ci), C.POINTER(vp), C.POINTER(vp), C.POINTER(vp)]
    L.T360B200_weightImage.restype = ci
    L.T360B200_weightImage.argtypes = [ci, C.POINTER(vp)]
    L.T360B200_remapTable.restype = ci
    L.T360B200_remapTable.argtypes = [ci, C.POINTER(vp)]
    L.T360B200_transformFramePlaneAsync.restype = ci
    L.T360B200_transformFramePlaneAsync.argtypes = [vp, vp, vp] + [ci] * 7 + [vp]
    L.T360B200_transformFrameAsync.restype = ci
    L.T360B200_transformFrameAsync.argtypes = [vp, ci, vp, vp] + [vp] * 6 + [vp]
    L.T360B200_lowPassPlaneAsync.restype = ci
    L.T360B200_lowPassPlaneAsync.argtypes = [vp, vp, vp] + [ci] * 5 + [vp]
    L.T360B200_reconfigure.restype = ci
    L.T360B200_reconfigure.argtypes = [vp, C.POINTER(FrameTransformContext)]
    L.T360B200_reconfigureAsync.restype = ci
    L.T360B200_reconfigureAsync.argtypes = [vp, C.POINTER(FrameTransformContext)]
    L.T360B200_reconfigureWait.restype = ci
    L.T360B200_reconfigureWait.argtypes = [vp, ci]
    L.T360B200_transformFrameViewAsync.restype = ci
    L.T360B200_transformFrameViewAsync.argtypes = [vp, C.POINTER(T360View), ci, vp, vp] + [vp] * 6 + [vp]
    L.T360B200_viewSamples.restype = ci
    L.T360B200_viewSamples.argtypes = [C.POINTER(FrameTransformContext), C.POINTER(T360View)] + [ci] * 4 + [vp]
    L.T360B200_transformFrameOrientedAsync.restype = ci
    L.T360B200_transformFrameOrientedAsync.argtypes = [vp, C.POINTER(T360Orientation), ci, vp, vp] + [vp] * 6 + [vp]
    L.T360B200_orientedSamples.restype = ci
    L.T360B200_orientedSamples.argtypes = [C.POINTER(FrameTransformContext), C.POINTER(T360Orientation)] + [ci] * 4 + [vp]
    L.T360B200_transformFramePoseAsync.restype = ci
    L.T360B200_transformFramePoseAsync.argtypes = [vp, C.POINTER(T360Pose), ci, vp, vp] + [vp] * 6 + [vp]
    L.T360B200_poseSamples.restype = ci
    L.T360B200_poseSamples.argtypes = [C.POINTER(FrameTransformContext), C.POINTER(T360Pose)] + [ci] * 4 + [vp]
    L.T360B200_lensMap.restype = ci
    L.T360B200_lensMap.argtypes = [C.POINTER(FrameTransformContext), C.POINTER(T360LensRig), C.POINTER(T360Orientation)] + [ci] * 4 + [vp]
    L.T360B200_transformFrameLensAsync.restype = ci
    L.T360B200_transformFrameLensAsync.argtypes = [vp, C.POINTER(T360LensRig), C.POINTER(T360Orientation), ci, vp, vp] + [vp] * 6 + [vp]
    L.T360B200_setPinHostPlanes.restype = None
    L.T360B200_setPinHostPlanes.argtypes = [vp, ci]
    L.T360B200_debugTrace.restype = None
    L.T360B200_debugTrace.argtypes = [vp, ci]
    L.T360B200_debugTraceRead.restype = C.c_ulonglong
    L.T360B200_debugTraceRead.argtypes = [vp, vp, C.c_ulonglong]
    L.T360B200_synchronize.restype = ci
    L.T360B200_synchronize.argtypes = [vp]
    L.T360B200_stream.restype = vp
    L.T360B200_stream.argtypes = [vp]
    L.T360B200_kernelLaunchCount.restype = C.c_ulonglong
    L.T360B200_planDeviceBytes.restype = C.c_ulonglong
    L.T360B200_planDeviceBytes.argtypes = [vp, ci]
    L.T360B200_planTileCounts.restype = ci
    L.T360B200_planTileCounts.argtypes = [vp, ci, C.POINTER(ci)]
    L.T360B200_deviceCount.restype = ci
    L.T360B200_version.restype = C.c_char_p
    if path is None:
        _lib = L
    return L


EXPORTED_SYMBOLS = [
    "VideoFrameTransform_new", "VideoFrameTransform_delete", "VideoFrameTransform_generateMapForPlane",
    "VideoFrameTransform_transformFramePlane", "T360B200_hostPlanCreate", "T360B200_hostPlanCreateFromWarp", "T360B200_hostPlanDestroy",
    "T360B200_generateMapFromWarp", "T360B200_remapFrameAsync",
    "T360B200_hostPlanInfo", "T360B200_hostPlanMap", "T360B200_hostPlanSamples", "T360B200_hostPlanSegment",
    "T360B200_hostPlanGather", "T360B200_hostPlanPoleCaps", "T360B200_hostPlanBlurLists", "T360B200_weightImage", "T360B200_dealLanes",
    "T360B200_remapTable", "T360B200_transformFramePlaneAsync", "T360B200_transformFrameAsync",
    "T360B200_lowPassPlaneAsync", "T360B200_reconfigure", "T360B200_reconfigureAsync", "T360B200_reconfigureWait",
    "T360B200_transformFrameViewAsync", "T360B200_viewSamples",
    "T360B200_transformFrameOrientedAsync", "T360B200_orientedSamples", "T360B200_transformFramePoseAsync", "T360B200_poseSamples",
    "T360B200_lensMap", "T360B200_transformFrameLensAsync",
    "T360B200_setPinHostPlanes", "T360B200_debugTrace", "T360B200_debugTraceRead", "T360B200_synchronize", "T360B200_stream", "T360B200_kernelLaunchCount", "T360B200_planDeviceBytes",
    "T360B200_planTileCounts", "T360B200_deviceCount", "T360B200_version",
]


class VideoFrameTransform:

    def __init__(self, ctx: FrameTransformContext):
        self._lib = load()
        self.ctx = ctx
        self._h = self._lib.VideoFrameTransform_new(C.byref(ctx))
        if not self._h:
            raise MemoryError("VideoFrameTransform_new returned NULL")

    def close(self):
        if getattr(self, "_h", None):
            self._lib.VideoFrameTransform_delete(self._h)
            self._h = None

    __del__ = close

    def __enter__(self):
        return self

    def __exit__(self, *exc):
        self.close()

    def generateMapForPlane(self, inputWidth, inputHeight, outputWidth, outputHeight, transformMatPlaneIndex) -> bool:
        return bool(self._lib.VideoFrameTransform_generateMapForPlane(
            self._h, inputWidth, inputHeight, outputWidth, outputHeight, transformMatPlaneIndex))

    def transformFramePlane(self, inputData, outputData, inputWidth, inputHeight, inputWidthWithPadding,
                            outputWidth, outputHeight, outputWidthWithPadding, transformMatPlaneIndex,
                            imagePlaneIndex) -> bool:
        return bool(self._lib.VideoFrameTransform_transformFramePlane(
            self._h, inputData, outputData, inputWidth, inputHeight, inputWidthWithPadding, outputWidth,
            outputHeight, outputWidthWithPadding, transformMatPlaneIndex, imagePlaneIndex))

    def transform_plane(self, src: np.ndarray, out_w: int, out_h: int, plan_index: int, image_plane: int = 0,
                        out: np.ndarray | None = None) -> np.ndarray:
        assert src.dtype == np.uint8 and src.ndim == 2 and src.strides[1] == 1
        if out is None:
            out = np.zeros((out_h, out_w), np.uint8)
        assert out.dtype == np.uint8 and out.shape == (out_h, out_w) and out.strides[1] == 1
        ok = self.transformFramePlane(src.ctypes.data, out.ctypes.data, src.shape[1], src.shape[0], src.strides[0],
                                      out_w, out_h, out.strides[0], plan_index, image_plane)
        if not ok:
            raise RuntimeError("VideoFrameTransform_transformFramePlane returned 0 (message on stdout)")
        return out

    def transform_plane_async(self, d_in: int, d_out: int, in_w, in_h, in_pitch, out_w, out_h, out_pitch, plan_index,
                              stream: int = 0) -> bool:
        return bool(self._lib.T360B200_transformFramePlaneAsync(self._h, d_in, d_out, in_w, in_h, in_pitch, out_w,
                                                                out_h, out_pitch, plan_index, stream))

    def make_frame_call(self, in_planes, out_planes, dims):
        n, pin, pout, ptrs, keep = _frame_args(in_planes, out_planes, dims)
        fn, h = self._lib.T360B200_transformFrameAsync, self._h

        def call(stream: int = 0, _keep=keep) -> bool:
            return bool(fn(h, n, pin, pout, *ptrs, stream))
        return call

    def make_view_frame_call(self, in_planes, out_planes, dims):
        n, pin, pout, ptrs, keep = _frame_args(in_planes, out_planes, dims)
        fn, h = self._lib.T360B200_transformFrameViewAsync, self._h

        def call(view, stream: int = 0, _keep=keep) -> bool:
            return bool(fn(h, C.byref(as_view(view)), n, pin, pout, *ptrs, stream))
        return call

    def make_oriented_frame_call(self, in_planes, out_planes, dims):
        n, pin, pout, ptrs, keep = _frame_args(in_planes, out_planes, dims)
        fn, h = self._lib.T360B200_transformFrameOrientedAsync, self._h

        def call(orientation, stream: int = 0, _keep=keep) -> bool:
            return bool(fn(h, C.byref(as_orientation(orientation)), n, pin, pout, *ptrs, stream))
        return call

    def make_pose_frame_call(self, in_planes, out_planes, dims):
        n, pin, pout, ptrs, keep = _frame_args(in_planes, out_planes, dims)
        fn, h = self._lib.T360B200_transformFramePoseAsync, self._h

        def call(pose, stream: int = 0, _keep=keep) -> bool:
            return bool(fn(h, C.byref(as_pose(pose)), n, pin, pout, *ptrs, stream))
        return call

    def make_lens_frame_call(self, in_planes, out_planes, dims):
        n, pin, pout, ptrs, keep = _frame_args(in_planes, out_planes, dims)
        fn, h = self._lib.T360B200_transformFrameLensAsync, self._h

        def call(rig, orientation, stream: int = 0, _keep=keep) -> bool:
            return bool(fn(h, C.byref(rig), C.byref(as_orientation(orientation)), n, pin, pout, *ptrs, stream))
        return call

    def generate_map_from_warp(self, map, in_w: int, in_h: int, plan_index: int, border: int = BORDER_WRAP) -> bool:
        m = _warp_map(map)
        return bool(self._lib.T360B200_generateMapFromWarp(self._h, m.ctypes.data, m.shape[1], m.shape[0], in_w, in_h, border,
                                                           plan_index))

    def make_remap_frame_call(self, in_planes, out_planes, dims, border: int = BORDER_WRAP):
        n, pin, pout, ptrs, keep = _frame_args(in_planes, out_planes, dims)
        fn, h = self._lib.T360B200_remapFrameAsync, self._h
        dense = [8 * d[2] for d in dims]

        def as_map(m, p):
            if hasattr(m, "data_ptr"):
                return m.data_ptr(), m.stride(0) * m.element_size()
            return (int(m[0]), int(m[1])) if isinstance(m, (tuple, list)) else (int(m), dense[p])

        def call(maps, stream: int = 0, _keep=keep) -> bool:
            if len(maps) != n:
                raise ValueError(f"{len(maps)} maps for {n} planes")
            desc = [as_map(m, p) for p, m in enumerate(maps)]
            dmaps, pitches = (C.c_void_p * n)(*[d[0] for d in desc]), (C.c_int * n)(*[d[1] for d in desc])
            return bool(fn(h, n, dmaps, pitches, border, pin, pout, *ptrs, stream))
        return call

    def low_pass_async(self, d_in: int, d_out: int, w, h, in_pitch, out_pitch, plan_index, stream: int = 0) -> bool:
        return bool(self._lib.T360B200_lowPassPlaneAsync(self._h, d_in, d_out, w, h, in_pitch, out_pitch, plan_index,
                                                         stream))

    def reconfigure(self, ctx: FrameTransformContext) -> None:
        if not self._lib.T360B200_reconfigure(self._h, C.byref(ctx)):
            raise RuntimeError("T360B200_reconfigure returned 0 (message on stdout); the old configuration is still in effect")
        self.ctx = ctx

    def reconfigure_async(self, ctx: FrameTransformContext) -> None:
        if not self._lib.T360B200_reconfigureAsync(self._h, C.byref(ctx)):
            raise RuntimeError("T360B200_reconfigureAsync returned 0 (message on stdout); the old context is still in effect")
        self.ctx = ctx

    def reconfigure_wait(self, block: bool = True) -> int:
        return self._lib.T360B200_reconfigureWait(self._h, 1 if block else 0)

    def set_pin_host_planes(self, enable: bool) -> None:
        self._lib.T360B200_setPinHostPlanes(self._h, 1 if enable else 0)

    def debug_trace(self, enable: bool) -> None:
        self._lib.T360B200_debugTrace(self._h, 1 if enable else 0)

    def read_trace(self) -> np.ndarray:
        buf = np.zeros(int(self._lib.T360B200_debugTraceRead(self._h, None, 0)), np.uint64)
        n = int(self._lib.T360B200_debugTraceRead(self._h, buf.ctypes.data, buf.size)) if buf.size else 0
        return buf[:n].reshape(-1, 64, 4)

    def synchronize(self) -> bool:
        return bool(self._lib.T360B200_synchronize(self._h))

    @property
    def stream(self) -> int:
        return self._lib.T360B200_stream(self._h) or 0

    def plan_tile_counts(self, plan_index):
        c = (C.c_int * 4)()
        if not self._lib.T360B200_planTileCounts(self._h, plan_index, c):
            raise KeyError(plan_index)
        return tuple(c)

    def plan_device_bytes(self, plan_index) -> int:
        return int(self._lib.T360B200_planDeviceBytes(self._h, plan_index))


class HostPlan:

    def __init__(self, ctx: FrameTransformContext, in_w, in_h, out_w, out_h, _handle=None):
        self._lib = load()
        self._h = _handle or self._lib.T360B200_hostPlanCreate(C.byref(ctx), in_w, in_h, out_w, out_h)
        if not self._h:
            raise ValueError("T360B200_hostPlanCreate failed (message on stdout)")
        info = (C.c_int * 6)()
        self._lib.T360B200_hostPlanInfo(self._h, info)
        self.map_w, self.map_h, self.num_segments, self.num_taps, self.kernel_size = info[0], info[1], info[2], info[3], info[4]

    @classmethod
    def from_warp(cls, ctx: FrameTransformContext, map, in_w, in_h, border: int = BORDER_WRAP) -> "HostPlan":
        m = _warp_map(map)
        h = load().T360B200_hostPlanCreateFromWarp(C.byref(ctx), m.ctypes.data, m.shape[1], m.shape[0], in_w, in_h, border)
        if not h:
            raise ValueError("T360B200_hostPlanCreateFromWarp failed (message on stdout)")
        return cls(ctx, in_w, in_h, m.shape[1], m.shape[0], _handle=h)

    def close(self):
        if getattr(self, "_h", None):
            self._lib.T360B200_hostPlanDestroy(self._h)
            self._h = None

    __del__ = close

    @property
    def map(self) -> np.ndarray:
        p = self._lib.T360B200_hostPlanMap(self._h)
        n = self.map_w * self.map_h * 2
        return np.frombuffer((C.c_float * n).from_address(p), np.float32).reshape(self.map_h, self.map_w, 2).copy()

    @property
    def samples(self) -> np.ndarray:
        p = self._lib.T360B200_hostPlanSamples(self._h)
        n = self.map_w * self.map_h * 2
        return np.frombuffer((C.c_int32 * n).from_address(p), np.int32).reshape(self.map_h, self.map_w, 2).copy()

    def gather_plan(self):
        info = (C.c_int * 10)()
        jobs, recs, comp = C.c_void_p(), C.c_void_p(), C.c_void_p()
        if not self._lib.T360B200_hostPlanGather(self._h, info, C.byref(jobs), C.byref(recs), C.byref(comp)):
            raise ValueError("T360B200_hostPlanGather failed")
        tpr, trows, th, nj = info[0], info[1], info[2], info[3]
        n = tpr * trows * th * 32 * 2
        records = np.frombuffer((C.c_int32 * n).from_address(recs.value), np.int32).reshape(tpr * trows, th, 32, 2).copy()
        j = compact = None
        if nj and jobs.value:
            j = np.frombuffer((C.c_int32 * (nj * 4)).from_address(jobs.value), np.int32).reshape(nj, 4).copy()
        if info[9] and comp.value:
            compact = np.frombuffer((C.c_uint32 * info[9]).from_address(comp.value), np.uint32).copy()
        return dict(tiles_per_row=tpr, tile_rows=trows, tile_h=th, jobs=j, records=records, compact=compact,
                    counts=dict(class0=info[4], class1=info[5], seam=info[6], general=info[7], share=info[8]))

    def pole_caps(self):
        info = (C.c_int * 4)()
        jobs, recs, launch = C.c_void_p(), C.c_void_p(), C.c_void_p()
        if not self._lib.T360B200_hostPlanPoleCaps(self._h, info, C.byref(jobs), C.byref(recs), C.byref(launch)):
            raise ValueError("T360B200_hostPlanPoleCaps failed")
        n, m = info[0] + info[1], info[3]
        as_jobs = lambda p, k: np.frombuffer((C.c_int32 * (k * 4)).from_address(p.value), np.int32).reshape(k, 4).copy() if k and p.value else np.zeros((0, 4), np.int32)
        records = np.frombuffer((C.c_uint32 * info[2]).from_address(recs.value), np.uint32).copy() if info[2] and recs.value else np.zeros(0, np.uint32)
        return dict(counts=dict(cap=info[0], border=info[1]), jobs=as_jobs(jobs, n), records=records, launch=as_jobs(launch, m))

    def blur_lists(self, *others, width=0, height=0):
        plans = (C.c_void_p * (1 + len(others)))(self._h, *[o._h for o in others])
        lay, img = (C.c_int * 15)(), C.c_void_p()
        if not self._lib.T360B200_hostPlanBlurLists(plans, len(plans), width, height, lay, C.byref(img)):
            raise ValueError("T360B200_hostPlanBlurLists failed (message on stdout)")
        image = C.string_at(img.value, lay[14]) if lay[14] else b""
        arr = lambda at, n, cols, dt: np.frombuffer(image, dt, n * cols, at).reshape(n, cols).copy()
        return dict(image=image, strips=[arr(lay[8 + c], lay[c], 9, np.int32) for c in range(3)], tiles=arr(lay[11], lay[3], 8, np.int32),
                    direct=arr(lay[12], lay[4], 8, np.int32), taps=np.frombuffer(image, np.float32, lay[5], lay[13]).copy(),
                    offsets=list(lay[8:14]), tile_smem=lay[6], needs_clear=bool(lay[7]))

    def segments(self):
        out = []
        rect, nk = (C.c_int * 4)(), (C.c_int * 2)()
        kx, ky = C.c_void_p(), C.c_void_p()
        for i in range(self.num_segments):
            assert self._lib.T360B200_hostPlanSegment(self._h, i, rect, nk, C.byref(kx), C.byref(ky))
            a = np.frombuffer((C.c_float * nk[0]).from_address(kx.value), np.float32).copy()
            b = np.frombuffer((C.c_float * nk[1]).from_address(ky.value), np.float32).copy()
            out.append((rect[0], rect[1], rect[2], rect[3], a, b))
        return out


def view_samples(ctx: FrameTransformContext, view, in_w, in_h, out_w, out_h) -> np.ndarray:
    return _samples(load().T360B200_viewSamples, ctx, as_view(view), in_w, in_h, out_w, out_h)


def oriented_samples(ctx: FrameTransformContext, orientation, in_w, in_h, out_w, out_h) -> np.ndarray:
    return _samples(load().T360B200_orientedSamples, ctx, as_orientation(orientation), in_w, in_h, out_w, out_h)


def pose_samples(ctx: FrameTransformContext, pose, in_w, in_h, out_w, out_h) -> np.ndarray:
    return _samples(load().T360B200_poseSamples, ctx, as_pose(pose), in_w, in_h, out_w, out_h)


def lens_map(ctx: FrameTransformContext, rig: T360LensRig, orientation, in_w, in_h, out_w, out_h) -> np.ndarray:
    out = np.zeros((max(out_h, 0), max(out_w, 0), 2), np.float32)
    if not load().T360B200_lensMap(C.byref(ctx), C.byref(rig), C.byref(as_orientation(orientation)), in_w, in_h, out_w, out_h,
                                   out.ctypes.data):
        raise ValueError("T360B200_lensMap refused the arguments (message on stdout)")
    return out


def remap_table(interpolation_alg: int) -> np.ndarray | None:
    L = load()
    p = C.c_void_p()
    k = L.T360B200_remapTable(interpolation_alg, C.byref(p))
    if k < 2:
        return None
    return np.frombuffer((C.c_int16 * (1024 * k * k)).from_address(p.value), np.int16).reshape(1024, k, k).copy()


def deal_lanes(interpolation_alg: int, phases) -> tuple[int, np.ndarray, np.ndarray]:
    L = load()
    ph = np.ascontiguousarray(phases, np.int32)
    lane, copy = np.zeros(ph.size, np.int32), np.zeros(ph.size, np.int32)
    L.T360B200_dealLanes.restype = C.c_int
    L.T360B200_dealLanes.argtypes = [C.c_int, C.c_int, C.c_void_p, C.c_void_p, C.c_void_p]
    w = L.T360B200_dealLanes(interpolation_alg, ph.size, ph.ctypes.data, lane.ctypes.data, copy.ctypes.data)
    if w < 0:
        raise ValueError("T360B200_dealLanes refused the arguments")
    return int(w), lane, copy


def weight_image(interpolation_alg: int) -> np.ndarray | None:
    L = load()
    p = C.c_void_p()
    n = L.T360B200_weightImage(interpolation_alg, C.byref(p))
    if n <= 0:
        return None
    return np.frombuffer((C.c_uint8 * n).from_address(p.value), np.uint8).copy()


def kernel_launch_count() -> int:
    return int(load().T360B200_kernelLaunchCount())


def device_count() -> int:
    return int(load().T360B200_deviceCount())
```

Before: 728,000.

## Use narrower TMA box widths for class-0 tile jobs based on footprint

Class-0 gather jobs now pick one of several TMA box widths (208/144/112/80 bytes) based on their actual column span, encoded in the top bits of the job's record offset. Host-side record offsets are rewritten to the narrower pitch, extra tensor maps are encoded per width, and the kernel dispatches computeTileJob over the width template. The aim is to cut bytes fetched into shared memory and reduce bank conflicts for jobs with small footprints. The cost is more tensor maps in the grid-constant parameters, extra template instantiations and branching, and a record-offset range limit. Bicubic uses kernel size 4, so all four widths apply to it.

Result: faster. 760,700, median of 6 (+4.5%).

```diff
diff --git a/include/transform360_b200.h b/include/transform360_b200.h
--- a/include/transform360_b200.h
+++ b/include/transform360_b200.h
@@ -23,6 +23,7 @@
                             const uint32_t** compact);
 int T360B200_hostPlanPoleCaps(T360HostPlan* plan, int info[4], const int32_t** capJobs, const uint32_t** capRecords,
                               const int32_t** launchJobs);
+int T360B200_hostPlanDeviceLists(T360HostPlan* plan, int info[2], const int32_t** jobs, const uint32_t** records);
 int T360B200_dealLanes(int interpolationAlg, int n, const int32_t* phases, int32_t* laneOf, int32_t* copyOf);
 int T360B200_weightImage(int interpolationAlg, const uint8_t** image);
 int T360B200_hostPlanBlurLists(T360HostPlan* const* plans, int numPlans, int width, int height, int layout[15],
diff --git a/profiles/box_footprint.py b/profiles/box_footprint.py
--- /dev/null
+++ b/profiles/box_footprint.py
@@ -0,0 +1,142 @@
+#!/usr/bin/env python
+import sys
+from pathlib import Path
+
+import numpy as np
+
+sys.path.insert(0, str(Path(__file__).resolve().parents[1]))
+import transform360_b200 as t360
+from tests.golden.cases import FULL, plane_dims
+
+KIND_SHIFT, SKIP, PITCH = 24, 0x8000, 208
+CLASS0, SHARE_STAY, SHARE, SEAM, CAP = 0, 3, 4, 7, 8
+SHARE_W = 192
+WIDTH_SETS = {"today": (208,), "2 widths": (112, 208), "3 widths": (80, 144, 208), "used": (80, 112, 144, 208),
+              "5 widths": (80, 112, 144, 176, 208)}
+USED = WIDTH_SETS["used"]
+
+
+def box_h(k, share):
+    return (80 if share else 72) if k == 8 else (72 if share else 64)
+
+
+def variant_rows(k, share, rows):
+    h = box_h(k, share)
+    heights = (h, h - 8, h - 16) if share else (h, h - 16, h - 24)
+    return min(v for v in heights if v >= rows)
+
+
+def plane_jobs(hp):
+    k = hp.kernel_size
+    g, pc = hp.gather_plan(), hp.pole_caps()
+    out, share_bytes = [], 0
+    if g["jobs"] is None:
+        return out, 0
+    compact = g["compact"]
+    for ox, oy, boxxy, rec in g["jobs"]:
+        kind = (int(oy) >> KIND_SHIFT) & 15
+        if kind in (SHARE, SHARE_STAY):
+            share_bytes += SHARE_W * (box_h(k, True) - 8 * (int(boxxy) & 15))
+            continue
+        if kind not in (CLASS0, SEAM):
+            continue
+        quad = (int(ox) & 7) - 1
+        n = 8 * 128 if quad < 0 else 4 * 64
+        words = compact[int(rec) * 4:int(rec) * 4 + n].astype(np.int64)
+        off = words[(words & SKIP) == 0] & 0x7FFF
+        name = "seam" if kind == SEAM else ("quad" if quad >= 0 else "tile")
+        out.append((name, int((off % PITCH).max()) + k, int((off // PITCH).max()) + k))
+    base = 0 if compact is None else compact.size // 4
+    for n, oy, boxxy, rec in pc["jobs"]:
+        if (int(oy) >> KIND_SHIFT) & 15 != CAP:
+            continue
+        w = pc["records"][(int(rec) - base) * 4:(int(rec) - base) * 4 + int(n) * 64].reshape(-1, 2)[:, 0].astype(np.int64)
+        off = w[(w & SKIP) == 0] & 0x7FFF
+        out.append(("cap", int((off % PITCH).max()) + k, int((off // PITCH).max()) + k))
+    return out, share_bytes
+
+
+def window_wavefronts(hp, widths):
+    from bank_sim import max_distinct_per_bank
+    k, g = hp.kernel_size, hp.gather_plan()
+    tot = {"208": 0, "narrow": 0}
+    n = 0
+    for ox, oy, boxxy, rec in g["jobs"][::97]:
+        if (int(oy) >> KIND_SHIFT) & 15 != CLASS0:
+            continue
+        quad = (int(ox) & 7) - 1
+        words = g["compact"][int(rec) * 4:int(rec) * 4 + (8 * 128 if quad < 0 else 4 * 64)].astype(np.int64)
+        words = words.reshape(8, 32, 4).transpose(0, 2, 1).reshape(-1, 32) if quad < 0 else words.reshape(4, 32, 2).transpose(0, 2, 1).reshape(-1, 32)
+        off = words & 0x7FFF
+        live = (words & SKIP) == 0
+        span = int((off[live] % PITCH).max()) + k
+        pitch = min(w for w in widths if w >= span)
+        for label, p in (("208", PITCH), ("narrow", pitch)):
+            moved = off - off // PITCH * (PITCH - p)
+            for step, ok in zip(moved, live):
+                if not ok.any():
+                    continue
+                for r in range(k):
+                    a = ((step[ok] & ~3) + r * p) // 4
+                    for extra in range(3 if k == 8 else 2):
+                        tot[label] += int(max_distinct_per_bank((a + extra)[None, :], 32)[0])
+                        n += label == "208"
+    return tot["208"] / max(n, 1), tot["narrow"] / max(n, 1)
+
+
+def box_bytes(jobs, k, widths, kinds=("tile", "quad")):
+    total = 0
+    for name, span, rows in jobs:
+        h = variant_rows(k, False, rows)
+        if name == "seam":
+            total += 2 * PITCH * h
+        elif name in kinds:
+            total += min(w for w in widths if w >= span) * h
+        else:
+            total += PITCH * h
+    return total
+
+
+def main():
+    for name in sys.argv[1:] or ["cfg2", "cfg4"]:
+        case = FULL[name]
+        ctx = t360.make_context(**case["ov"])
+        frame, share = [], 0
+        for plane, copies in ((0, 1), (1, 2)):
+            iw, ih, ow, oh, _ = plane_dims(case, plane)
+            hp = t360.HostPlan(ctx, iw, ih, ow, oh)
+            k = hp.kernel_size
+            jobs, sb = plane_jobs(hp)
+            frame += jobs * copies
+            share += sb * copies
+            if plane == 0:
+                bank = window_wavefronts(hp, USED)
+            hp.close()
+        print(f"{name}: kernel size {k}, {len(frame)} class-0 box jobs per frame (Y + U + V)")
+        for kind in ("tile", "quad", "cap", "seam"):
+            span = np.array([s for n, s, _ in frame if n == kind])
+            rows = np.array([r for n, _, r in frame if n == kind])
+            if not span.size:
+                continue
+            q = np.percentile(span, [10, 50, 90, 100]).astype(int)
+            hist = np.bincount(np.minimum(span, 208) // 16, minlength=14)[1:14]
+            print(f"  {kind:4s} {span.size:5d} jobs  span bytes p10/p50/p90/max {q[0]}/{q[1]}/{q[2]}/{q[3]}  rows p50/max "
+                  f"{int(np.median(rows))}/{rows.max()}")
+            print(f"       span bytes in 16-byte steps (16 .. 208): {' '.join(str(int(v)) for v in hist)}")
+        polar = [j for j in frame if j[0] in ("tile", "quad")]
+        used = np.array([min(w for w in USED if w >= s) for n, s, _ in polar])
+        print("  tiles and quadrants per width of " + str(USED) + ": " +
+              " / ".join(f"{100 * (used == w).mean():.0f} %" for w in USED))
+        print(f"  window loads of the luma tiles and quadrants (bank model, wavefronts per 32-bit load): "
+              f"{bank[0]:.2f} at 208 B, {bank[1]:.2f} in the narrow boxes")
+        today = box_bytes(frame, k, (208,))
+        print(f"  share-job boxes {share / 1e6:.2f} MB per frame; class-0 box jobs:")
+        for label, widths in WIDTH_SETS.items():
+            b = box_bytes(frame, k, widths)
+            p0, p1 = box_bytes(polar, k, (208,)), box_bytes(polar, k, widths)
+            print(f"    {label:6s} {str(widths):22s} {b / 1e6:6.2f} MB per frame ({100 * (1 - b / today):4.1f} % less; "
+                  f"the tiles and quadrants alone {p0 / 1e6:.2f} -> {p1 / 1e6:.2f} MB, {100 * (1 - p1 / p0):4.1f} % less)")
+
+
+if __name__ == "__main__":
+    main()
diff --git a/transform360_b200/csrc/gather_frame.cu b/transform360_b200/csrc/gather_frame.cu
--- a/transform360_b200/csrc/gather_frame.cu
+++ b/transform360_b200/csrc/gather_frame.cu
@@ -256,8 +256,9 @@
   }
 }
 
+template <int K>
 struct FrameTensorMaps {
-  CUtensorMap map[kMaxFramePlanes][kNumBoxClasses][kBoxVariants];
+  CUtensorMap map[kMaxFramePlanes][boxMaps(K)];
 };
 
 __device__ __forceinline__ void mbarArrive(uint64_t* bar) {
@@ -290,7 +291,7 @@
 
 template <int K, int COPIES, int GROUPS>
 __global__ void __launch_bounds__(GROUPS * (kGroupWarps + 1) * 32, 1)
-gatherFrameKernel(const __grid_constant__ FrameGatherParams p, StagedParams jobs, const __grid_constant__ FrameTensorMaps maps) {
+gatherFrameKernel(const __grid_constant__ FrameGatherParams p, StagedParams jobs, const __grid_constant__ FrameTensorMaps<K> maps) {
   using L = FrameLayout<K, COPIES, GROUPS>;
   constexpr int VS = weightVectorStride(K, COPIES), kStage = L::kStage, kRec = L::kRec, S = L::kStages;
   constexpr uint32_t kBox0 = stageBoxW(K, 0) * stageBoxH(K, 0), kBox1 = stageBoxW(K, 1) * stageBoxH(K, 1),
@@ -382,13 +383,14 @@
             mbarExpectTx(full + st, recBytes);
           } else {
             const int cls = boxClassOf(kind), variant = jobBoxVariant(h.z), boxX = jobBoxX(h.z), boxY = jobBoxY(h.z);
-            const uint32_t boxBytes = (uint32_t)(stageBoxW(K, cls) * boxVariantRows(K, cls, variant));
+            const int width = (int)((unsigned)h.w >> kJobWidthShift);
+            const uint32_t boxBytes = (uint32_t)((cls == 0 ? class0BoxW(width) : stageBoxW(K, cls)) * boxVariantRows(K, cls, variant));
             mbarExpectTx(full + st, (kind == kJobSeam ? 2 : 1) * boxBytes + recBytes);
-            tmaLoadBox(groupBase + st * kStage, &maps.map[pl][cls][variant], boxX, boxY, full + st);
+            tmaLoadBox(groupBase + st * kStage, &maps.map[pl][boxMapIndex(K, cls, width, variant)], boxX, boxY, full + st);
             if (kind == kJobSeam)
-              tmaLoadBox(groupBase + (st + 1) * kStage, &maps.map[pl][0][variant], boxX - planes[pl].srcW, boxY, full + st);
+              tmaLoadBox(groupBase + (st + 1) * kStage, &maps.map[pl][boxMapIndex(K, 0, 0, variant)], boxX - planes[pl].srcW, boxY, full + st);
           }
-          bulkCopyToShared(rec + 128, planes[pl].records + (unsigned)h.w, recBytes, full + st);
+          bulkCopyToShared(rec + 128, planes[pl].records + ((unsigned)h.w & kJobRecordMask), recBytes, full + st);
         }
       }
       advance();
@@ -452,7 +454,11 @@
           if (quad & 1) { r.z = v.x; r.w = v.y; } else { r.x = v.x; r.y = v.y; }
         }
       }
-      computeTileJob<K, stageBoxW(K, 0), VS>(pv, boxAddr + st * kStage, outX, outY, r, wAddr, warp);
+      const int width = (int)(h.w >> kJobWidthShift);
+      staticFor<class0Widths(K)>([&](auto W) {
+        constexpr int w = decltype(W)::value;
+        if (width == w) computeTileJob<K, class0BoxW(w), VS>(pv, boxAddr + st * kStage, outX, outY, r, wAddr, warp);
+      });
     } else if (kind == kJobClass1) {
       computeTileJob<K, stageBoxW(K, 1), VS>(pv, boxAddr + st * kStage, outX, outY, ldsVec(rec + 128 + warp * 512 + lane * 16), wAddr, warp);
     } else if (kind == kJobSeam) {
@@ -492,8 +498,12 @@
 }
 
 template <int K, int COPIES, int GROUPS>
-cudaError_t launchFrameK(const FrameGatherParams& p, const StagedParams& jobs, const FrameTensorMaps& maps, int numSMs,
+cudaError_t launchFrameK(const FrameGatherParams& p, const StagedParams& jobs, const void* tensorMaps, int numSMs,
                          cudaStream_t stream, bool programmatic) {
+  FrameTensorMaps<K> maps;
+  for (int i = 0; i < kMaxFramePlanes; ++i)
+    std::memcpy(maps.map[i], static_cast<const CUtensorMap*>(tensorMaps) + (size_t)(i < p.numPlanes ? i : 0) * kMaxBoxMaps,
+                sizeof(maps.map[i]));
   constexpr int threads = GROUPS * (kGroupWarps + 1) * 32, smemBytes = FrameLayout<K, COPIES, GROUPS>::kTotal;
   LaunchCfg cfg;
   cudaError_t err = prepareFrameK<K, COPIES, GROUPS>(cfg);
@@ -530,15 +540,10 @@
                               cudaStream_t stream, bool programmatic) {
   if (jobs.numTiles <= 0) return cudaSuccess;
   if (p.numPlanes < 1 || p.numPlanes > kMaxFramePlanes) return cudaErrorInvalidValue;
-  FrameTensorMaps maps;
-  std::memcpy(&maps, tensorMaps, sizeof(CUtensorMap) * kNumBoxClasses * kBoxVariants * p.numPlanes);
-  for (int i = p.numPlanes; i < kMaxFramePlanes; ++i)
-    for (int c = 0; c < kNumBoxClasses; ++c)
-      for (int v = 0; v < kBoxVariants; ++v) maps.map[i][c][v] = maps.map[0][c][v];
   switch (p.kernelSize) {
-    case 2: return launchFrameK<2, weightCopies(2), gatherGroups(2)>(p, jobs, maps, numSMs, stream, programmatic);
-    case 4: return launchFrameK<4, weightCopies(4), gatherGroups(4)>(p, jobs, maps, numSMs, stream, programmatic);
-    case 8: return launchFrameK<8, weightCopies(8), gatherGroups(8)>(p, jobs, maps, numSMs, stream, programmatic);
+    case 2: return launchFrameK<2, weightCopies(2), gatherGroups(2)>(p, jobs, tensorMaps, numSMs, stream, programmatic);
+    case 4: return launchFrameK<4, weightCopies(4), gatherGroups(4)>(p, jobs, tensorMaps, numSMs, stream, programmatic);
+    case 8: return launchFrameK<8, weightCopies(8), gatherGroups(8)>(p, jobs, tensorMaps, numSMs, stream, programmatic);
     default: return cudaErrorInvalidValue;
   }
 }
diff --git a/transform360_b200/csrc/gather_plan.cpp b/transform360_b200/csrc/gather_plan.cpp
--- a/transform360_b200/csrc/gather_plan.cpp
+++ b/transform360_b200/csrc/gather_plan.cpp
@@ -609,6 +609,7 @@
   g.compact.assign(offset / 4, 0u);
   std::vector<int> needRows(g.jobs.size(), h.inH);
   std::vector<JobRect> rects(g.jobs.size());
+  std::vector<uint8_t> widths(g.jobs.size(), 0);
   parallelRanges(static_cast<int>(g.jobs.size()), 2048, [&](int begin, int end) {
     for (int i = begin; i < end; ++i) {
       const GatherJob& job = g.jobs[i];
@@ -620,6 +621,7 @@
       if (kind == kJobGeneral) continue;
       const Extent e = extentOf(h, r.x0, r.y0, r.x1, r.y1);
       if (e.minR >= 0 && e.maxR + k <= h.inH) needRows[i] = e.maxR + k;
+      if (kind == kJobClass0) widths[i] = static_cast<uint8_t>(class0WidthFor(k, e.maxC + k - jobBoxX(job.boxXY)));
       uint32_t* out = g.compact.data() + static_cast<size_t>(job.recordOffset) * 4;
       if (boxClassOf(kind) == 2) writeShareRecords(h, job, out);
       else writeTileRecords(h, job, out);
@@ -647,7 +649,33 @@
     g.launchJobs.push_back(jobOf(i));
     g.launchNeedRows.push_back(i >= 0 ? needRows[i] : pixelJobs[-1 - i].needRows);
     g.launchRects.push_back(i >= 0 ? rects[i] : pixelJobs[-1 - i].rect);
-  }
-}
-
-}
+    g.launchBoxWidths.push_back(i >= 0 ? widths[i] : 0);
+  }
+  if (offset / 16 > static_cast<size_t>(kJobRecordMask)) throw std::invalid_argument("gather plan: too many sampling records");
+}
+
+std::vector<GatherJob> deviceJobs(const GatherPlan& g) {
+  std::vector<GatherJob> out(g.launchJobs);
+  for (size_t i = 0; i < out.size(); ++i) out[i].recordOffset |= static_cast<int>(g.launchBoxWidths[i]) << kJobWidthShift;
+  return out;
+}
+
+std::vector<uint32_t> deviceRecords(const GatherPlan& g, int k) {
+  std::vector<uint32_t> out(g.compact);
+  out.insert(out.end(), g.capRecords.begin(), g.capRecords.end());
+  const int wide = stageBoxW(k, 0);
+  for (size_t i = 0; i < g.launchJobs.size(); ++i) {
+    if (g.launchBoxWidths[i] == 0) continue;
+    const GatherJob& job = g.launchJobs[i];
+    const uint32_t narrow = static_cast<uint32_t>(class0BoxW(g.launchBoxWidths[i]));
+    uint32_t* w = out.data() + static_cast<size_t>(job.recordOffset) * 4;
+    for (int j = 0; j < jobRecordBytes(k, kJobClass0, job.outX) / 4; ++j) {
+      if (w[j] & kRecordSkip) continue;
+      const uint32_t off = w[j] & 0x7fffu;
+      w[j] = (w[j] & ~0x7fffu) | (off / wide * narrow + off % wide);
+    }
+  }
+  return out;
+}
+
+}
diff --git a/transform360_b200/csrc/gather_plan.h b/transform360_b200/csrc/gather_plan.h
--- a/transform360_b200/csrc/gather_plan.h
+++ b/transform360_b200/csrc/gather_plan.h
@@ -22,11 +22,15 @@
   std::vector<GatherJob> launchJobs;
   std::vector<int> launchNeedRows;
   std::vector<JobRect> launchRects;
+  std::vector<uint8_t> launchBoxWidths;
   int numStaged[2] = {}, numSeam = 0, numGeneral = 0, numShare = 0, numCap = 0, numBorder = 0;
   int totalStaged() const { return numSeam + numShare + numStaged[0] + numStaged[1] + numCap; }
 };
 
 void buildGatherPlan(const HostPlan& h, bool stageTiles, GatherPlan& g);
+
+std::vector<GatherJob> deviceJobs(const GatherPlan& g);
+std::vector<uint32_t> deviceRecords(const GatherPlan& g, int k);
 
 inline int jobLaunchRank(const GatherJob& job) {
   switch ((job.outY >> kJobKindShift) & kJobKindMask) {
diff --git a/transform360_b200/csrc/kernels.cuh b/transform360_b200/csrc/kernels.cuh
--- a/transform360_b200/csrc/kernels.cuh
+++ b/transform360_b200/csrc/kernels.cuh
@@ -64,6 +64,29 @@
   while (v + 1 < kBoxVariants && cls != 1 && boxVariantRows(k, cls, v + 1) >= rows) ++v;
   return v;
 }
+constexpr int kClass0Widths = 4, kJobWidthShift = 28, kJobRecordMask = (1 << kJobWidthShift) - 1;
+__host__ __device__ constexpr int class0BoxW(int w) { return w == 0 ? 208 : (w == 1 ? 144 : (w == 2 ? 112 : 80)); }
+__host__ __device__ constexpr int class0Widths(int k) { return k == 8 ? 1 : kClass0Widths; }
+__host__ __device__ constexpr int class0WidthFor(int k, int cols) {
+  int w = 0;
+  while (w + 1 < class0Widths(k) && class0BoxW(w + 1) >= cols) ++w;
+  return w;
+}
+__host__ __device__ constexpr int boxMaps(int k) { return class0Widths(k) * kBoxVariants + 1 + kBoxVariants; }
+constexpr int kMaxBoxMaps = kClass0Widths * kBoxVariants + 1 + kBoxVariants;
+__host__ __device__ constexpr int boxMapIndex(int k, int cls, int width, int variant) {
+  return cls == 0 ? width * kBoxVariants + variant : (cls == 1 ? class0Widths(k) * kBoxVariants : class0Widths(k) * kBoxVariants + 1 + variant);
+}
+__host__ __device__ constexpr int boxMapClass(int k, int i) {
+  return i < class0Widths(k) * kBoxVariants ? 0 : (i == class0Widths(k) * kBoxVariants ? 1 : 2);
+}
+__host__ __device__ constexpr int boxMapW(int k, int i) { return boxMapClass(k, i) == 0 ? class0BoxW(i / kBoxVariants) : stageBoxW(k, boxMapClass(k, i)); }
+__host__ __device__ constexpr int boxMapRows(int k, int i) {
+  return boxMapClass(k, i) == 0 ? boxVariantRows(k, 0, i % kBoxVariants)
+         : boxMapClass(k, i) == 1 ? stageBoxH(k, 1)
+                                  : boxVariantRows(k, 2, i - class0Widths(k) * kBoxVariants - 1);
+}
+
 __host__ __device__ constexpr int gatherStages(int ) { return 2; }
 __host__ __device__ constexpr int stageBytesOf(int k) {
   const int a = stageBoxW(k, 2) * stageBoxH(k, 2), b = stageBoxW(k, 0) * stageBoxH(k, 0);
diff --git a/transform360_b200/csrc/video_frame_transform.cpp b/transform360_b200/csrc/video_frame_transform.cpp
--- a/transform360_b200/csrc/video_frame_transform.cpp
+++ b/transform360_b200/csrc/video_frame_transform.cpp
@@ -175,13 +175,13 @@
   return fn;
 }
 
-bool encodePlaneMap(CUtensorMap* map, const uint8_t* base, int w, int h, int pitch, int k, int cls, int variant) {
+bool encodePlaneMap(CUtensorMap* map, const uint8_t* base, int w, int h, int pitch, int k, int index) {
   EncodeTiledFn enc = tensorMapEncoder();
   if (!enc) return false;
   if ((reinterpret_cast<uintptr_t>(base) & 15) || (pitch & 15)) return false;
   const cuuint64_t dims[2] = {static_cast<cuuint64_t>(w), static_cast<cuuint64_t>(h)};
   const cuuint64_t strides[1] = {static_cast<cuuint64_t>(pitch)};
-  const cuuint32_t box[2] = {static_cast<cuuint32_t>(t360::stageBoxW(k, cls)), static_cast<cuuint32_t>(t360::boxVariantRows(k, cls, variant))};
+  const cuuint32_t box[2] = {static_cast<cuuint32_t>(t360::boxMapW(k, index)), static_cast<cuuint32_t>(t360::boxMapRows(k, index))};
   const cuuint32_t elem[2] = {1, 1};
   return enc(map, CU_TENSOR_MAP_DATA_TYPE_UINT8, 2, const_cast<uint8_t*>(base), dims, strides, box, elem,
              CU_TENSOR_MAP_INTERLEAVE_NONE, CU_TENSOR_MAP_SWIZZLE_NONE, CU_TENSOR_MAP_L2_PROMOTION_L2_128B,
@@ -193,7 +193,7 @@
 struct PlaneMaps {
   const uint8_t* base = nullptr;
   int w = 0, h = 0, pitch = 0, k = 0;
-  CUtensorMap maps[t360::kNumBoxClasses][t360::kBoxVariants];
+  CUtensorMap maps[t360::kMaxBoxMaps];
 };
 struct PlaneLane {
   static constexpr int kMapCache = 32;
@@ -210,7 +210,7 @@
   const DevicePlan* plan = nullptr;
   t360::PlaneView view{};
   bool staged = false;
-  CUtensorMap maps[t360::kNumBoxClasses][t360::kBoxVariants];
+  CUtensorMap maps[t360::kMaxBoxMaps];
   uint8_t* finalOut = nullptr;
   int finalPitch = 0, finalW = 0, finalH = 0, imagePlane = 0;
   const void* resizeTables = nullptr;
@@ -1377,18 +1377,16 @@
       d.numStaged = g.totalStaged();
       d.numBorder = g.numBorder;
       d.numJobs = static_cast<int>(g.launchJobs.size());
-      if (!g.launchJobs.empty()) {
-        d.gatherJobs.reserve(g.launchJobs.size());
-        CU(cudaMemcpy(d.gatherJobs.ptr, g.launchJobs.data(), g.launchJobs.size() * sizeof(GatherJob), cudaMemcpyHostToDevice));
+      d.hostJobs = t360::deviceJobs(g);
+      if (!d.hostJobs.empty()) {
+        d.gatherJobs.reserve(d.hostJobs.size());
+        CU(cudaMemcpy(d.gatherJobs.ptr, d.hostJobs.data(), d.hostJobs.size() * sizeof(GatherJob), cudaMemcpyHostToDevice));
       }
       if (!g.compact.empty() || !g.capRecords.empty()) {
-        d.records.reserve(g.compact.size() + g.capRecords.size());
-        if (!g.compact.empty())
-          CU(cudaMemcpy(d.records.ptr, g.compact.data(), g.compact.size() * sizeof(uint32_t), cudaMemcpyHostToDevice));
-        if (!g.capRecords.empty())
-          CU(cudaMemcpy(d.records.ptr + g.compact.size(), g.capRecords.data(), g.capRecords.size() * sizeof(uint32_t), cudaMemcpyHostToDevice));
-      }
-      d.hostJobs = std::move(g.launchJobs);
+        const std::vector<uint32_t> records = t360::deviceRecords(g, d.kernelSize);
+        d.records.reserve(records.size());
+        CU(cudaMemcpy(d.records.ptr, records.data(), records.size() * sizeof(uint32_t), cudaMemcpyHostToDevice));
+      }
       d.jobNeedRows = std::move(g.launchNeedRows);
       d.jobRects = std::move(g.launchRects);
     }
@@ -1504,21 +1502,15 @@
   }
 
   static bool planeMaps(PlaneLane& lane, const uint8_t* src, int w, int h, int pitch, int k,
-                        CUtensorMap (&out)[t360::kNumBoxClasses][t360::kBoxVariants]) {
+                        CUtensorMap (&out)[t360::kMaxBoxMaps]) {
     for (const PlaneMaps& e : lane.mapCache)
       if (e.base == src && e.w == w && e.h == h && e.pitch == pitch && e.k == k) {
         std::memcpy(out, e.maps, sizeof(e.maps));
         return true;
       }
     PlaneMaps fresh;
-    for (int c = 0; c < t360::kNumBoxClasses; ++c)
-      for (int v = 0; v < t360::kBoxVariants; ++v) {
-        if (v > 0 && t360::boxVariantRows(k, c, v) == t360::boxVariantRows(k, c, 0)) {
-          fresh.maps[c][v] = fresh.maps[c][0];
-          continue;
-        }
-        if (!encodePlaneMap(&fresh.maps[c][v], src, w, h, pitch, k, c, v)) return false;
-      }
+    for (int m = 0; m < t360::boxMaps(k); ++m)
+      if (!encodePlaneMap(&fresh.maps[m], src, w, h, pitch, k, m)) return false;
     fresh.base = src; fresh.w = w; fresh.h = h; fresh.pitch = pitch; fresh.k = k;
     lane.mapCache[lane.mapCacheNext] = fresh;
     lane.mapCacheNext = (lane.mapCacheNext + 1) % PlaneLane::kMapCache;
@@ -1772,7 +1764,7 @@
     const FrameListRefs f = frameLists(plans, numPlanes);
     armScheduler(slot.frameClaim, s);
     t360::FrameGatherParams fp{};
-    CUtensorMap maps[kPlaneLanes][t360::kNumBoxClasses][t360::kBoxVariants];
+    CUtensorMap maps[kPlaneLanes][t360::kMaxBoxMaps];
     for (int p = 0; p < numPlanes; ++p) {
       fp.plane[p] = work[p].view;
       std::memcpy(maps[p], work[p].maps, sizeof(work[p].maps));
@@ -2113,6 +2105,8 @@
   HostPlan plan;
   t360::GatherPlan gather;
   bool gatherBuilt = false;
+  std::vector<GatherJob> deviceJobs;
+  std::vector<uint32_t> deviceRecords;
   std::vector<uint8_t> blurImage;
 };
 
@@ -2186,6 +2180,20 @@
   if (capJobs) *capJobs = g.capJobs.empty() ? nullptr : reinterpret_cast<const int32_t*>(g.capJobs.data());
   if (capRecords) *capRecords = g.capRecords.empty() ? nullptr : g.capRecords.data();
   if (launchJobs) *launchJobs = g.launchJobs.empty() ? nullptr : reinterpret_cast<const int32_t*>(g.launchJobs.data());
+  return 1;
+}
+T360_API int T360B200_hostPlanDeviceLists(T360HostPlan* plan, int info[2], const int32_t** jobs, const uint32_t** records) {
+  int gatherInfo[10];
+  if (!plan || !info || !jobs || !records || !T360B200_hostPlanGather(plan, gatherInfo, nullptr, nullptr, nullptr)) return 0;
+  const t360::GatherPlan& g = plan->gather;
+  if (plan->deviceJobs.size() != g.launchJobs.size()) {
+    plan->deviceJobs = t360::deviceJobs(g);
+    plan->deviceRecords = t360::deviceRecords(g, plan->plan.kernelSize);
+  }
+  info[0] = static_cast<int>(plan->deviceJobs.size());
+  info[1] = static_cast<int>(plan->deviceRecords.size());
+  *jobs = plan->deviceJobs.empty() ? nullptr : reinterpret_cast<const int32_t*>(plan->deviceJobs.data());
+  *records = plan->deviceRecords.empty() ? nullptr : plan->deviceRecords.data();
   return 1;
 }
 T360_API int T360B200_hostPlanBlurLists(T360HostPlan* const* plans, int numPlans, int width, int height, int layout[15],
diff --git a/transform360_b200/handler.py b/transform360_b200/handler.py
--- a/transform360_b200/handler.py
+++ b/transform360_b200/handler.py
@@ -160,6 +160,8 @@
     L.T360B200_hostPlanBlurLists.restype = ci
     L.T360B200_hostPlanBlurLists.argtypes = [vp, ci, ci, ci, C.POINTER(ci), C.POINTER(vp)]
     L.T360B200_hostPlanPoleCaps.argtypes = [vp, C.POINTER(ci), C.POINTER(vp), C.POINTER(vp), C.POINTER(vp)]
+    L.T360B200_hostPlanDeviceLists.restype = ci
+    L.T360B200_hostPlanDeviceLists.argtypes = [vp, C.POINTER(ci), C.POINTER(vp), C.POINTER(vp)]
     L.T360B200_weightImage.restype = ci
     L.T360B200_weightImage.argtypes = [ci, C.POINTER(vp)]
     L.T360B200_remapTable.restype = ci
@@ -219,7 +221,7 @@
     "VideoFrameTransform_transformFramePlane", "T360B200_hostPlanCreate", "T360B200_hostPlanCreateFromWarp", "T360B200_hostPlanDestroy",
     "T360B200_generateMapFromWarp", "T360B200_remapFrameAsync",
     "T360B200_hostPlanInfo", "T360B200_hostPlanMap", "T360B200_hostPlanSamples", "T360B200_hostPlanSegment",
-    "T360B200_hostPlanGather", "T360B200_hostPlanPoleCaps", "T360B200_hostPlanBlurLists", "T360B200_weightImage", "T360B200_dealLanes",
+    "T360B200_hostPlanGather", "T360B200_hostPlanPoleCaps", "T360B200_hostPlanDeviceLists", "T360B200_hostPlanBlurLists", "T360B200_weightImage", "T360B200_dealLanes",
     "T360B200_remapTable", "T360B200_transformFramePlaneAsync", "T360B200_transformFrameAsync",
     "T360B200_lowPassPlaneAsync", "T360B200_reconfigure", "T360B200_reconfigureAsync", "T360B200_reconfigureWait",
     "T360B200_transformFrameViewAsync", "T360B200_viewSamples",
@@ -452,6 +454,15 @@
         records = np.frombuffer((C.c_uint32 * info[2]).from_address(recs.value), np.uint32).copy() if info[2] and recs.value else np.zeros(0, np.uint32)
         return dict(counts=dict(cap=info[0], border=info[1]), jobs=as_jobs(jobs, n), records=records, launch=as_jobs(launch, m))
 
+    def device_lists(self):
+        info = (C.c_int * 2)()
+        jobs, recs = C.c_void_p(), C.c_void_p()
+        if not self._lib.T360B200_hostPlanDeviceLists(self._h, info, C.byref(jobs), C.byref(recs)):
+            raise ValueError("T360B200_hostPlanDeviceLists failed")
+        j = np.frombuffer((C.c_int32 * (info[0] * 4)).from_address(jobs.value), np.int32).reshape(-1, 4).copy() if info[0] and jobs.value else np.zeros((0, 4), np.int32)
+        r = np.frombuffer((C.c_uint32 * info[1]).from_address(recs.value), np.uint32).copy() if info[1] and recs.value else np.zeros(0, np.uint32)
+        return dict(jobs=j, records=r)
+
     def blur_lists(self, *others, width=0, height=0):
         plans = (C.c_void_p * (1 + len(others)))(self._h, *[o._h for o in others])
         lay, img = (C.c_int * 15)(), C.c_void_p()
```
